# gautam-sabnis/A-Divide-and-Conquer-Strategy-for-High-Dimensional-Bayesian-Factor-Models

Measured on AMD Instinct MI355X. Metric: Gibbs iters/sec (node) at p=20k,n=1k,g=64; cov-assembly MFMA util %, higher is better.
Workload: dtype f64; 1 GPU; c3: p=19968 (P=312 x g=64), n=1000, K=30 (k=1920), rho=0.5, thin=5, burnin=0 (assembly in timed region), asm_batch=96; global_batch=1000, parallelism=shards64/gpus1

## Files before the change

### a-divide-and-conquer-strategy-for-high-dimensional-bayesian-factor-models_amd/_abi.py

```python
from __future__ import annotations

import ctypes as C
import os
from pathlib import Path

PKG_DIR = Path(__file__).resolve().parent
LIB_PATH = Path(os.environ.get("DCFM_LIB", PKG_DIR / "libdcfm.so"))

DCFM_OK = 0
DCFM_ERR_INVALID = 1
DCFM_ERR_UNSUPPORTED = 2
DCFM_ERR_HIP = 3
DCFM_ERR_RCCL = 4
DCFM_ERR_NUMERIC = 5
DCFM_ERR_ALLOC = 6
DCFM_FLAG_INJECT_DRAWS = 0x1
DCFM_FLAG_UNFUSED = 0x2
DCFM_FLAG_ONE_STREAM = 0x4
DCFM_FLAG_FLAT_PRIORITY = 0x8
DCFM_FLAG_COMM_SELF = 0x20
DCFM_FLAG_EXACT_RESIDUAL = 0x10
DCFM_FLAG_GUARD_ALL = 0x40
DCFM_FLAG_SIGMA_M2 = 0x80
DCFM_FLAG_PRECISION_MEAN = 0x100
DCFM_FLAG_PARTIAL_CORR = 0x200
DCFM_SIGMA_MEAN = 0
DCFM_SIGMA_M2 = 1
DCFM_SIGMA_SD = 2
SIGMA_MOMENTS = {"mean": DCFM_SIGMA_MEAN, "m2": DCFM_SIGMA_M2, "sd": DCFM_SIGMA_SD}

KERNEL_IDS = {
    "k_prep": 0, "k_wpass": 1, "k_zdraw": 2, "k_xred": 3, "k_xdraw": 4, "k_cpass": 5,
    "k_lambda": 6, "k_colsum": 7, "k_delta": 8, "k_save": 9, "k_assemble": 10, "rccl": 11,
    "k_xchol": 12, "k_draws": 13, "k_resid": 14,
}
K_COUNT = 15

EXPORTS = (
    "dcfm_create", "dcfm_destroy", "dcfm_last_error", "dcfm_abi_version",
    "dcfm_comm_unique_id", "dcfm_comm_init", "dcfm_comm_init_loopback", "dcfm_set_data", "dcfm_set_state",
    "dcfm_set_draws", "dcfm_run", "dcfm_synchronize", "dcfm_get_state", "dcfm_get_state_raw", "dcfm_get_sigma",
    "dcfm_get_sigma_cols", "dcfm_sigma_block", "dcfm_get_sigma_moment_cols", "dcfm_get_sigma_moment",
    "dcfm_saved_samples", "dcfm_sigma_error", "dcfm_set_profiling", "dcfm_set_profiling_mask", "dcfm_set_profiling_stride", "dcfm_get_kernel_stats",
    "dcfm_kernel_name",
    "dcfm_rng_fill", "dcfm_rng_fill_rows", "dcfm_set_data_raw", "dcfm_get_data", "dcfm_count_nonzero_columns",
    "dcfm_set_trace", "dcfm_get_trace", "dcfm_init_state", "dcfm_sigma_apply", "dcfm_sigma_eigs",
    "dcfm_sigma_solve", "dcfm_set_probes", "dcfm_get_probe_draws", "dcfm_set_precision_probes",
    "dcfm_get_precision_draws", "dcfm_get_precision_mean_cols", "dcfm_get_precision_mean",
    "dcfm_get_partial_corr_cols", "dcfm_get_partial_corr",
    "dcfm_set_loglik", "dcfm_get_loglik", "dcfm_set_predict", "dcfm_get_predict",
    "dcfm_set_missing", "dcfm_get_imputed",
)


class DcfmConfig(C.Structure):
    _fields_ = [
        ("n", C.c_int32), ("P", C.c_int32), ("g", C.c_int32), ("K", C.c_int32),
        ("rho", C.c_double),
        ("burnin", C.c_int64), ("mcmc", C.c_int64), ("thin", C.c_int64),
        ("as_", C.c_double), ("bs", C.c_double), ("df", C.c_double), ("ad1", C.c_double),
        ("bd1", C.c_double), ("ad2", C.c_double), ("bd2", C.c_double),
        ("seed", C.c_uint64),
        ("nranks", C.c_int32), ("rank", C.c_int32), ("device", C.c_int32),
        ("flags", C.c_uint32), ("asm_batch", C.c_int32), ("reserved", C.c_int32 * 7),
    ]


_DP = C.POINTER(C.c_double)


class DcfmStateView(C.Structure):
    _fields_ = [(f, _DP) for f in ("Lambda", "ps", "omega", "psi", "Plam", "X", "Z", "eta", "delta", "tauh")]


class DcfmDrawsView(C.Structure):
    _fields_ = [(f, _DP) for f in ("NZ", "NX", "NL", "Gpsi", "Gdelta", "Gps")]


class DcfmError(RuntimeError):
    def __init__(self, code: int, msg: str):
        super().__init__(f"dcfm error {code}: {msg}")
        self.code = code


_lib = None


def load_library(path: Path | None = None):
    global _lib
    if _lib is not None:
        return _lib
    p = Path(path) if path else LIB_PATH
    if not p.exists():
        raise ImportError(
            f"libdcfm.so not found at {p}: build it first (python -c 'import __graft_entry__ as g; g.build()' "
            "or make -C <pkg>/csrc). There is no CPU fallback.")
    lib = C.CDLL(str(p))
    vp = C.c_void_p
    sig = {
        "dcfm_create": (C.c_int, [C.POINTER(DcfmConfig), C.POINTER(vp)]),
        "dcfm_destroy": (None, [vp]),
        "dcfm_last_error": (C.c_char_p, [vp]),
        "dcfm_abi_version": (C.c_int, []),
        "dcfm_comm_unique_id": (C.c_int, [C.POINTER(C.c_uint8)]),
        "dcfm_comm_init": (C.c_int, [vp, C.POINTER(C.c_uint8)]),
        "dcfm_comm_init_loopback": (C.c_int, [C.POINTER(vp), C.c_int32]),
        "dcfm_set_data": (C.c_int, [vp, _DP]),
        "dcfm_set_state": (C.c_int, [vp, C.POINTER(DcfmStateView)]),
        "dcfm_set_draws": (C.c_int, [vp, C.POINTER(DcfmDrawsView), C.c_int64, C.c_int64]),
        "dcfm_run": (C.c_int, [vp, C.c_int64, C.c_int64]),
        "dcfm_synchronize": (C.c_int, [vp]),
        "dcfm_get_state": (C.c_int, [vp, C.POINTER(DcfmStateView)]),
        "dcfm_get_state_raw": (C.c_int, [vp, C.POINTER(DcfmStateView)]),
        "dcfm_get_sigma": (C.c_int, [vp, _DP]),
        "dcfm_get_sigma_cols": (C.c_int, [vp, C.c_int64, C.c_int64, _DP]),
        "dcfm_sigma_block": (C.c_int, [vp, C.POINTER(C.c_int64)]),
        "dcfm_get_sigma_moment_cols": (C.c_int, [vp, C.c_int32, C.c_int64, C.c_int64, _DP]),
        "dcfm_get_sigma_moment": (C.c_int, [vp, C.c_int32, _DP]),
        "dcfm_get_precision_mean_cols": (C.c_int, [vp, C.c_int64, C.c_int64, _DP]),
        "dcfm_get_precision_mean": (C.c_int, [vp, _DP]),
        "dcfm_get_partial_corr_cols": (C.c_int, [vp, C.c_int32, C.c_int64, C.c_int64, _DP]),
        "dcfm_get_partial_corr": (C.c_int, [vp, C.c_int32, _DP]),
        "dcfm_saved_samples": (C.c_int64, [vp]),
        "dcfm_sigma_error": (C.c_int, [vp, _DP, C.c_int32, _DP, C.c_int32, C.c_uint64, _DP]),
        "dcfm_sigma_apply": (C.c_int, [vp, _DP, C.c_int32, _DP, _DP]),
        "dcfm_sigma_eigs": (C.c_int, [vp, C.c_int32, C.c_double, C.c_int32, C.c_uint64, _DP, _DP, _DP,
                                      C.POINTER(C.c_int32)]),
        "dcfm_sigma_solve": (C.c_int, [vp, _DP, C.c_int32, C.c_double, C.c_int32, _DP, _DP, C.POINTER(C.c_int32),
                                       _DP, _DP]),
        "dcfm_set_probes": (C.c_int, [vp, _DP, C.c_int32, C.c_int64]),
        "dcfm_get_probe_draws": (C.c_int, [vp, _DP, C.POINTER(C.c_int64)]),
        "dcfm_set_precision_probes": (C.c_int, [vp, _DP, C.c_int32, C.c_int64]),
        "dcfm_get_precision_draws": (C.c_int, [vp, _DP, _DP, C.POINTER(C.c_int64)]),
        "dcfm_set_loglik": (C.c_int, [vp, C.c_int64]),
        "dcfm_get_loglik": (C.c_int, [vp, _DP, _DP, C.POINTER(C.c_int64)]),
        "dcfm_set_predict": (C.c_int, [vp, _DP, C.POINTER(C.c_uint8), C.c_int32, C.c_int64]),
        "dcfm_get_predict": (C.c_int, [vp, _DP, _DP, _DP, _DP, _DP, C.POINTER(C.c_int64)]),
        "dcfm_set_missing": (C.c_int, [vp, C.POINTER(C.c_uint8), C.c_int64]),
        "dcfm_get_imputed": (C.c_int, [vp, _DP, _DP, _DP, C.POINTER(C.c_int64)]),
        "dcfm_set_profiling": (C.c_int, [vp, C.c_int]),
        "dcfm_set_profiling_mask": (C.c_int, [vp, C.c_uint32]),
        "dcfm_set_profiling_stride": (C.c_int, [vp, C.c_int32]),
        "dcfm_get_kernel_stats": (C.c_int, [vp, _DP, C.POINTER(C.c_int64)]),
        "dcfm_kernel_name": (C.c_char_p, [C.c_int]),
        "dcfm_rng_fill": (C.c_int, [C.c_int, C.c_uint64, C.c_int, C.c_double, C.c_int32, C.c_int32,
                                    C.c_int64, C.c_int64, _DP]),
        "dcfm_rng_fill_rows": (C.c_int, [C.c_int, C.c_uint64, C.c_int, C.c_double, C.c_int32, C.c_int32,
                                         C.c_int64, C.c_int64, C.c_int32, C.c_int64, _DP]),
        "dcfm_set_data_raw": (C.c_int, [vp, _DP, C.c_int64, C.POINTER(C.c_int64), _DP, _DP]),
        "dcfm_get_data": (C.c_int, [vp, _DP]),
        "dcfm_set_trace": (C.c_int, [vp, C.c_int64]),
        "dcfm_init_state": (C.c_int, [vp]),
        "dcfm_get_trace": (C.c_int, [vp, _DP, C.POINTER(C.c_int64)]),
        "dcfm_count_nonzero_columns": (C.c_int, [C.c_int, _DP, C.c_int32, C.c_int64, C.POINTER(C.c_int32),
                                                 _DP]),
    }
    for name, (res, args) in sig.items():
        fn = getattr(lib, name)
        fn.restype = res
        fn.argtypes = args
    _lib = lib
    return lib


def check(lib, handle, code: int):
    if code != DCFM_OK:
        msg = lib.dcfm_last_error(handle)
        raise DcfmError(code, msg.decode() if msg else "")
```

### a-divide-and-conquer-strategy-for-high-dimensional-bayesian-factor-models_amd/csrc/dcfm.hip

```cpp
#include "handle.h"
#include "resid.h"

static int dalloc(dcfm_handle *h, double **p, size_t n) {
    void *q = nullptr;
    if (n == 0) n = 1;
    hipError_t e = hipMalloc(&q, n * sizeof(double));
    if (e != hipSuccess)
        return fail(h, DCFM_ERR_ALLOC, "hipMalloc(%zu doubles) failed: %s", n, hipGetErrorString(e));
    e = hipMemset(q, 0, n * sizeof(double));
    if (e != hipSuccess) return fail(h, DCFM_ERR_HIP, "hipMemset failed: %s", hipGetErrorString(e));
    h->allocs.push_back(q);
    *p = static_cast<double *>(q);
    return DCFM_OK;
}

static int round_up(int a, int b) { return (a + b - 1) / b * b; }

static double *trace_row(dcfm_handle *h, int64_t t) {
    return h->trace + trace_scratch_doubles(h->d.G) + (size_t)t * h->d.G * 4;
}

static void collect_prof(dcfm_handle *h) {
    if (h->recs.empty()) return;
    sync_all(h);
    for (auto &r : h->recs) {
        float ms = 0.f;
        if (hipEventElapsedTime(&ms, r.a, r.b) == hipSuccess) {
            h->kms[r.kid] += ms;
            h->kcnt[r.kid] += 1;
        }
        h->evpool.push_back(r.a);
        h->evpool.push_back(r.b);
    }
    h->recs.clear();
}

static std::vector<int> sigma_split(int nt, int nranks) {
    std::vector<int> Tb(nranks + 1, nt);
    Tb[0] = 0;
    const double total = (double)tri(nt);
    for (int k = 1; k < nranks; ++k) {
        const double target = total * k / nranks;
        int t = Tb[k - 1];
        while (t < nt && (double)tri(t) < target) ++t;
        if (t > Tb[k - 1] && target - (double)tri(t - 1) < (double)tri(t) - target) --t;
        Tb[k] = t;
    }
    return Tb;
}

extern "C" {

int dcfm_abi_version(void) { return DCFM_ABI_VERSION; }

const char *dcfm_last_error(const dcfm_handle *h) { return h ? h->err.c_str() : g_err.c_str(); }

const char *dcfm_kernel_name(int id) {
    static const char *names[DCFM_K_COUNT] = {"k_prep",  "k_wpass", "k_zdraw",  "k_xred",
                                              "k_xdraw", "k_cpass", "k_lambda", "k_colsum",
                                              "k_delta", "k_save",  "k_assemble", "rccl", "k_xchol",
                                              "k_draws", "k_resid"};
    return (id >= 0 && id < DCFM_K_COUNT) ? names[id] : "?";
}

static int validate_config(const dcfm_config &c) {
    if (c.n < 1 || c.P < 1 || c.g < 1 || c.K < 1)
        return fail(nullptr, DCFM_ERR_INVALID, "n, P, g, K must be >= 1");
    if (c.K > KP_MAX)
        return fail(nullptr, DCFM_ERR_UNSUPPORTED, "K = %d > %d not supported by this build", c.K, KP_MAX);
    if (!(c.rho >= 0.0 && c.rho <= 1.0)) return fail(nullptr, DCFM_ERR_INVALID, "rho must be in [0,1]");
    if (c.thin < 1 || c.mcmc < 0 || c.burnin < 0)
        return fail(nullptr, DCFM_ERR_INVALID, "thin >= 1, mcmc >= 0, burnin >= 0 required");
    if (!(c.bs > 0 && c.bd1 > 0 && c.bd2 > 0 && c.df > 0))
        return fail(nullptr, DCFM_ERR_INVALID, "bs, bd1, bd2, df must be > 0 (dc:62-65)");
    if (!(c.as_ > 0.0 && c.ad1 > 0.0 && c.ad2 > 0.0))
        return fail(nullptr, DCFM_ERR_INVALID, "as, ad1, ad2 must be > 0 (dc:62-65; got %g, %g, %g)", c.as_, c.ad1,
                    c.ad2);
    const int nranks = c.nranks < 1 ? 1 : c.nranks;
    if (c.rank < 0 || c.rank >= nranks) return fail(nullptr, DCFM_ERR_INVALID, "bad rank");
    {
        const bool fused = c.K <= KP && !(c.flags & DCFM_FLAG_UNFUSED);
        const int Gl = c.g / nranks, nxs = xsum_blocks(Gl);
        if (fused && (c.g > 1023 || nxs > 255 || Gl / nxs > 255))
            return fail(nullptr, DCFM_ERR_UNSUPPORTED, "g = %d shards (%d per rank): the fused K <= 32 chain takes at "
                        "most 1023, and a per-rank count whose odd part is below 256 (DCFM_FLAG_UNFUSED lifts "
                        "this)", c.g, Gl);
        if (!fused && c.g >= (1 << 16))
            return fail(nullptr, DCFM_ERR_UNSUPPORTED, "g = %d shards: at most %d", c.g, (1 << 16) - 1);
    }
    if (c.g % nranks)
        return fail(nullptr, DCFM_ERR_UNSUPPORTED, "g = %d not divisible by nranks = %d", c.g, nranks);
    return DCFM_OK;
}

static Dims plan(const dcfm_config &c, bool *fused, int *B, int *LDB) {
    Dims d{};
    const int nranks = c.nranks < 1 ? 1 : c.nranks;
    d.n = c.n; d.P = c.P; d.g = c.g; d.K = c.K;
    d.nranks = nranks; d.rank = c.rank;
    d.coll = (nranks > 1 || (c.flags & DCFM_FLAG_COMM_SELF)) ? 1 : 0;
    d.G = c.g / nranks;
    d.shard0 = c.rank * d.G;
    d.NP = round_up(c.n, 128);
    d.PP = round_up(c.P, 32);
    d.p = c.P * c.g;
    d.kp = padded_width(c.K);
    d.rho = c.rho; d.sr = std::sqrt(c.rho); d.s1r = std::sqrt(1.0 - c.rho);
    d.as_ = c.as_; d.bs = c.bs; d.df = c.df; d.ad1 = c.ad1; d.bd1 = c.bd1; d.ad2 = c.ad2; d.bd2 = c.bd2;
    d.seed = c.seed;
    d.inject = (c.flags & DCFM_FLAG_INJECT_DRAWS) ? 1 : 0;
    *fused = d.kp == KP && !(c.flags & DCFM_FLAG_UNFUSED);
    const bool packed = d.coll && *fused;
    d.sgap = packed ? KP * KP + d.NP * KP : 0;
    d.xstride = packed ? d.G * KP + KP * KP + d.NP * KP : d.kp * d.kp;
    *B = c.asm_batch > 0 ? c.asm_batch : 32;
    *LDB = round_up(*B * d.K, ASM_KC);
    return d;
}

static int create_streams_and_events(dcfm_handle *h) {
    const dcfm_config &c = h->cfg;
    HIPC(h, hipSetDevice(c.device));
    int prio_lo = 0, prio_hi = 0;
    if (!(c.flags & DCFM_FLAG_FLAT_PRIORITY)) HIPC(h, hipDeviceGetStreamPriorityRange(&prio_lo, &prio_hi));
    HIPC(h, hipStreamCreateWithPriority(&h->stream, hipStreamNonBlocking, prio_hi));
    {
        if (c.flags & DCFM_FLAG_ONE_STREAM) {
            h->side = h->sasm = h->sdraw = h->stream;
        } else {
            HIPC(h, hipStreamCreateWithPriority(&h->side, hipStreamNonBlocking, prio_hi));
            HIPC(h, hipStreamCreateWithPriority(&h->sdraw, hipStreamNonBlocking, prio_lo));
            HIPC(h, hipStreamCreateWithPriority(&h->sasm, hipStreamNonBlocking, prio_lo));
        }
    }
    for (hipEvent_t *e : {&h->e_lam, &h->e_prep, &h->e_xchol, &h->e_batch, &h->e_free[0], &h->e_free[1], &h->e_drawn[0],
                          &h->e_used[0], &h->e_drawn[1], &h->e_used[1]})
        HIPC(h, hipEventCreateWithFlags(e, hipEventDisableTiming));
    return DCFM_OK;
}

static int alloc_buffers(dcfm_handle *h) {
    const dcfm_config &c = h->cfg;
    const int nranks = c.nranks;
    void *q = nullptr;
    HIPC(h, hipMalloc(&q, sizeof(int)));
    h->allocs.push_back(q);
    h->nan_dev = static_cast<int *>(q);
    HIPC(h, hipMemset(h->nan_dev, 0, sizeof(int)));
    HIPC(h, hipHostMalloc(&q, sizeof(int), hipHostMallocDefault));
    h->nan_host = static_cast<int *>(q);
    *h->nan_host = 0;
    const Dims &d = h->d;
    Bufs &b = h->b;
    const size_t G = d.G, NP = d.NP, PP = d.PP, g = d.g, p = d.p, KP = d.kp;
    TRY(dalloc(h, &b.Y, G * NP * PP));
    TRY(dalloc(h, &b.yy, G * PP));
    TRY(dalloc(h, &b.Lam, G * PP * KP));
    TRY(dalloc(h, &b.omega, G * PP));
    TRY(dalloc(h, &b.ps, G * PP));
    TRY(dalloc(h, &b.psi, G * PP * KP));
    TRY(dalloc(h, &b.Plam, G * PP * KP));
    TRY(dalloc(h, &b.X, NP * KP));
    TRY(dalloc(h, &b.Z, G * NP * KP));
    TRY(dalloc(h, &b.delta, 2 * g * KP));
    TRY(dalloc(h, &b.tau, 2 * g * KP));
    TRY(dalloc(h, &b.W, G * NP * KP));
    TRY(dalloc(h, &b.A, G * KP * KP));
    TRY(dalloc(h, &b.ZM, G * 4 * KP * KP));
    TRY(dalloc(h, &b.Sp, G * NP * KP));
    if (d.sgap) {
        const size_t msg = (size_t)d.xstride;
        TRY(dalloc(h, &b.sloc, msg));
        b.xa = b.sloc + (size_t)G * KP;
        b.xin = b.xa + KP * KP;
        TRY(dalloc(h, &b.msg_all, (size_t)nranks * msg));
        b.sall = b.msg_all;
        b.xa_all = b.msg_all + (size_t)G * KP;
        b.xall = b.xa_all + KP * KP;
    } else {
        TRY(dalloc(h, &b.xin, NP * KP));
        if (d.coll) { TRY(dalloc(h, &b.xall, (size_t)nranks * NP * KP)); } else b.xall = b.xin;
        TRY(dalloc(h, &b.xa, KP * KP));
        TRY(dalloc(h, &b.xa_all, (size_t)nranks * KP * KP));
    }
    TRY(dalloc(h, &b.XM, 2 * KP * KP));
    TRY(dalloc(h, &b.agree, 3));
    {
        double *rf = nullptr;
        TRY(dalloc(h, &rf, (G * (PP / 32) + 1) / 2));
        b.rflag = reinterpret_cast<int *>(rf);
    }
    TRY(dalloc(h, &b.xpart, (size_t)G * KP * KP));
    {
        double *tk = nullptr;
        TRY(dalloc(h, &tk, 1));
        b.ticket = reinterpret_cast<unsigned *>(tk);
        double *sy = nullptr;
        TRY(dalloc(h, &sy, SYNC_ZM + G));
        b.sync = reinterpret_cast<unsigned long long *>(sy);
    }
    TRY(dalloc(h, &b.C, G * PP * KP));
    TRY(dalloc(h, &b.E, G * KP * KP));
    TRY(dalloc(h, &b.cpart, G * PP * KP));
    if (!d.sgap) {
        TRY(dalloc(h, &b.sloc, G * KP));
        if (d.coll) { TRY(dalloc(h, &b.sall, g * KP)); } else b.sall = b.sloc;
    }
    TRY(dalloc(h, &b.Lb[0], p * (size_t)b.LDB));
    TRY(dalloc(h, &b.Lb[1], p * (size_t)b.LDB));
    TRY(dalloc(h, &b.wsum[0], p));
    TRY(dalloc(h, &b.wsum[1], p));
    {
        const int nt = (d.p + ASM_TILE - 1) / ASM_TILE;
        h->Tb = sigma_split(nt, nranks);
        b.T0 = h->Tb[c.rank];
        b.T1 = h->Tb[c.rank + 1];
    }
    TRY(dalloc(h, &b.Sigma, (size_t)(tri(b.T1) - tri(b.T0)) * ASM_TILE * ASM_TILE));
    if (c.flags & DCFM_FLAG_SIGMA_M2) {
        TRY(dalloc(h, &b.Sigma2, (size_t)(tri(b.T1) - tri(b.T0)) * ASM_TILE * ASM_TILE));
    }
    if (c.flags & DCFM_FLAG_PRECISION_MEAN)
        TRY(dalloc(h, &h->pm.Prec, (size_t)(tri(b.T1) - tri(b.T0)) * ASM_TILE * ASM_TILE));
    if (c.flags & DCFM_FLAG_PARTIAL_CORR) {
        TRY(dalloc(h, &h->pc.PC, (size_t)(tri(b.T1) - tri(b.T0)) * ASM_TILE * ASM_TILE));
        TRY(dalloc(h, &h->pc.PC2, (size_t)(tri(b.T1) - tri(b.T0)) * ASM_TILE * ASM_TILE));
    }
    if (c.flags & (DCFM_FLAG_PRECISION_MEAN | DCFM_FLAG_PARTIAL_CORR)) {
        PrecMean &pm = h->pm;
        pm.KH = round_up(h->B * d.K, ASM_KC);
        TRY(dalloc(h, &pm.pfac, p * 4 * (size_t)pm.KH));
        TRY(dalloc(h, &pm.pscr, precision_mean_scratch_doubles(d.g, d.K, h->B)));
        HIPC(h, precision_mean_setup());
    }
    if (c.flags & (DCFM_FLAG_SIGMA_M2 | DCFM_FLAG_PRECISION_MEAN | DCFM_FLAG_PARTIAL_CORR)) {
        TRY(dalloc(h, &b.wslot[0], p * (size_t)h->B));
        TRY(dalloc(h, &b.wslot[1], p * (size_t)h->B));
    }
    if (h->fused && !d.inject) TRY(dalloc(h, &b.ldraw, (size_t)lam_gen_doubles(d)));
    if (!d.inject && !h->fused) {
        const size_t K = c.K, n = c.n, P = c.P;
        const size_t nz = K * n * g, nx = K * n, nl = K * P * g, gpsi = P * K * g, gdel = K * g, gps = P * g;
        const size_t per_it = nz + nx + nl + gpsi + gdel + gps;
        h->DB = (int)std::max<size_t>(1, std::min<size_t>(8, (size_t(2) << 30) / (2 * per_it * sizeof(double))));
        const size_t sz[6] = {nz, nx, nl, gpsi, gdel, gps};
        for (int i = 0; i < 6; ++i) h->draw_iter_sz[i] = sz[i];
        double *gm = nullptr;
        TRY(dalloc(h, &gm, 2 * (size_t)h->DB * per_it));
        for (int sl = 0; sl < 2; ++sl) {
            DrawsDev &G = h->gen[sl];
            G.NZ = gm; gm += nz * h->DB;
            G.NX = gm; gm += nx * h->DB;
            G.NL = gm; gm += nl * h->DB;
            G.Gpsi = gm; gm += gpsi * h->DB;
            G.Gdelta = gm; gm += gdel * h->DB;
            G.Gps = gm; gm += gps * h->DB;
            G.first_iter = -1;
            G.n_iter = h->DB;
        }
    }
    return DCFM_OK;
}

static int upload_tile_list(dcfm_handle *h) {
    Bufs &b = h->b;
    constexpr int SB = 8;
    std::vector<int2> tl;
    for (int rb0 = b.T0; rb0 < b.T1; rb0 += SB) {
        const int rb1 = std::min(b.T1, rb0 + SB);
        for (int cb0 = 0; cb0 < rb1; cb0 += SB)
            for (int ti = rb0; ti < rb1; ++ti)
                for (int tj = cb0; tj < std::min(cb0 + SB, ti + 1); ++tj) tl.push_back(make_int2(ti, tj));
    }
    if ((int64_t)tl.size() != tri(b.T1) - tri(b.T0))
        return fail(h, DCFM_ERR_INVALID, "assembly tile list: %zu tiles for %lld", tl.size(),
                    (long long)(tri(b.T1) - tri(b.T0)));
    b.ntiles = (int)tl.size();
    void *q = nullptr;
    HIPC(h, hipMalloc(&q, std::max<size_t>(1, tl.size()) * sizeof(int2)));
    h->allocs.push_back(q);
    b.tiles = static_cast<int2 *>(q);
    if (!tl.empty()) HIPC(h, hipMemcpy(b.tiles, tl.data(), tl.size() * sizeof(int2), hipMemcpyHostToDevice));
    return DCFM_OK;
}

static int fill_delta_tau_ones(dcfm_handle *h) {
    std::vector<double> ones(2 * (size_t)h->d.g * h->d.kp, 1.0);
    HIPC(h, hipMemcpy(h->b.delta, ones.data(), ones.size() * sizeof(double), hipMemcpyHostToDevice));
    HIPC(h, hipMemcpy(h->b.tau, ones.data(), ones.size() * sizeof(double), hipMemcpyHostToDevice));
    return DCFM_OK;
}

int dcfm_create(const dcfm_config *cfg, dcfm_handle **out) {
    if (!cfg || !out) return fail(nullptr, DCFM_ERR_INVALID, "null argument");
    *out = nullptr;
    const dcfm_config &c = *cfg;
    TRY(validate_config(c));
    int ndev = 0;
    hipError_t e = hipGetDeviceCount(&ndev);
    if (e != hipSuccess || ndev < 1)
        return fail(nullptr, DCFM_ERR_HIP, "no HIP device available (%s)", hipGetErrorString(e));
    if (c.device < 0 || c.device >= ndev) return fail(nullptr, DCFM_ERR_INVALID, "bad device %d", c.device);

    dcfm_handle *h = new dcfm_handle();
    h->d = plan(c, &h->fused, &h->B, &h->b.LDB);
    h->cfg = c;
    h->cfg.nranks = h->d.nranks;
    int rc = create_streams_and_events(h);
    if (rc == DCFM_OK) rc = alloc_buffers(h);
    if (rc == DCFM_OK) rc = upload_tile_list(h);
    if (rc == DCFM_OK) rc = fill_delta_tau_ones(h);
    if (rc != DCFM_OK) {
        g_err = h->err;
        dcfm_destroy(h);
        return rc;
    }
    *out = h;
    return DCFM_OK;
}

void dcfm_destroy(dcfm_handle *h) {
    if (!h) return;
    (void)hipSetDevice(h->cfg.device);
    if (h->stream) sync_all(h);
    for (auto &r : h->recs) { (void)hipEventDestroy(r.a); (void)hipEventDestroy(r.b); }
    for (auto e : h->evpool) (void)hipEventDestroy(e);
    for (hipEvent_t e : {h->e_lam, h->e_prep, h->e_xchol, h->e_batch, h->e_free[0], h->e_free[1], h->e_drawn[0],
                         h->e_drawn[1], h->e_used[0], h->e_used[1]})
        if (e) (void)hipEventDestroy(e);
    if (h->lp_ready) (void)hipEventDestroy(h->lp_ready);
    if (h->lp_done) (void)hipEventDestroy(h->lp_done);
    if (h->comm_asm) ncclCommDestroy(h->comm_asm);
    if (h->comm_side) ncclCommDestroy(h->comm_side);
    if (h->comm) ncclCommDestroy(h->comm);
    for (void *q : h->allocs) (void)hipFree(q);
    if (h->nan_host) (void)hipHostFree(h->nan_host);
    if (h->draws_mem) (void)hipFree(h->draws_mem);
    if (h->trace) (void)hipFree(h->trace);
    if (h->probe_mem) (void)hipFree(h->probe_mem);
    if (h->prec_mem) (void)hipFree(h->prec_mem);
    if (h->ll_mem) (void)hipFree(h->ll_mem);
    if (h->pred_mem) (void)hipFree(h->pred_mem);
    if (h->imp_mem) (void)hipFree(h->imp_mem);
    if (h->sasm && h->sasm != h->stream) (void)hipStreamDestroy(h->sasm);
    if (h->side && h->side != h->stream) (void)hipStreamDestroy(h->side);
    if (h->sdraw && h->sdraw != h->stream) (void)hipStreamDestroy(h->sdraw);
    if (h->stream) (void)hipStreamDestroy(h->stream);
    delete h;
}

static int flush_batch(dcfm_handle *h) {
    if (h->batch == 0) return DCFM_OK;
    Dims &d = h->d;
    Bufs &b = h->b;
    const int lb = h->lb;
    HIPC(h, hipEventRecord(h->e_batch, h->stream));
    HIPC(h, hipStreamWaitEvent(h->sasm, h->e_batch, 0));
    if (d.coll) {
        KTimer t(h, DCFM_K_COMM, h->sasm);
        const size_t rows = (size_t)d.G * d.P;
        if (!h->loop) NCCLC(h, ncclGroupStart());
        int rc = coll_allgather(h, CH_ASM, b.Lb[lb] + (size_t)d.rank * rows * b.LDB, b.Lb[lb], rows * b.LDB,
                                h->sasm);
        if (rc == DCFM_OK)
            rc = coll_allgather(h, CH_ASM, b.wsum[lb] + (size_t)d.rank * rows, b.wsum[lb], rows, h->sasm);
        if (rc == DCFM_OK && b.wslot[lb])
            rc = coll_allgather(h, CH_ASM, b.wslot[lb] + (size_t)d.rank * rows * h->B, b.wslot[lb], rows * h->B,
                                h->sasm);
        if (!h->loop) NCCLC(h, ncclGroupEnd());
        if (rc) return rc;
    }
    const int used = h->batch * d.K, kext = round_up(used, 4), kstage = round_up(used, ASM_KC);
    const double effsamp = (double)h->cfg.mcmc / (double)h->cfg.thin;
    if (kstage > used)
        HIPC(h, hipMemset2DAsync(b.Lb[lb] + used, (size_t)b.LDB * sizeof(double), 0, (size_t)(kstage - used) * sizeof(double),
                                 (size_t)d.p, h->sasm));
    {
        KTimer t(h, DCFM_K_ASSEMBLE, h->sasm);
        launch_assemble(d, b, b.Lb[lb], b.wsum[lb], kext, 1.0 / effsamp, h->sasm);
        if (b.Sigma2) launch_assemble_m2(d, b, b.Lb[lb], b.wslot[lb], h->batch, h->B, 1.0 / effsamp, h->sasm);
        if (h->pm.pfac) launch_precision_panels(d, b, h->pm, b.Lb[lb], b.wslot[lb], h->batch, h->B, h->sasm);
        if (h->pm.Prec) launch_precision_mean(d, b, h->pm, b.wslot[lb], h->batch, h->B, 1.0 / effsamp, h->sasm);
        if (h->pc.PC) launch_partial_corr(d, b, h->pm, h->pc, b.wslot[lb], h->batch, h->B, 1.0 / effsamp, h->sasm);
    }
    HIPC(h, hipGetLastError());
    HIPC(h, hipMemsetAsync(b.wsum[lb], 0, (size_t)d.p * sizeof(double), h->sasm));
    HIPC(h, hipEventRecord(h->e_free[lb], h->sasm));
    h->asm_pending[lb] = true;
    h->lb ^= 1;
    h->batch = 0;
    return DCFM_OK;
}

static int check_run_args(dcfm_handle *h, int64_t first_iter, int64_t n_iter) {
    if (!h) return fail(h, DCFM_ERR_INVALID, "null handle");
    if (!h->have_data || !h->have_state) return fail(h, DCFM_ERR_INVALID, "set_data and set_state first");
    if (first_iter < 1 || n_iter < 0) return fail(h, DCFM_ERR_INVALID, "iterations are 1-based");
    if (h->d.coll && !h->comm_ok) return fail(h, DCFM_ERR_INVALID, "dcfm_comm_init first (nranks > 1 or COMM_SELF)");
    if (h->d.inject) {
        if (!h->dr.NZ) return fail(h, DCFM_ERR_INVALID, "INJECT_DRAWS set but no draws");
        if (first_iter < h->dr.first_iter || first_iter + n_iter > h->dr.first_iter + h->dr.n_iter)
            return fail(h, DCFM_ERR_INVALID, "iterations [%lld,%lld) not covered by injected draws",
                        (long long)first_iter, (long long)(first_iter + n_iter));
    }
    return DCFM_OK;
}

struct DeltaTau { const double *delta_in, *tau_in; double *delta_out, *tau_out; };
static DeltaTau delta_tau(const dcfm_handle *h) {
    const size_t nkg = (size_t)h->d.g * h->d.kp, in = h->cur * nkg, out = (1 - h->cur) * nkg;
    return {h->b.delta + in, h->b.tau + in, h->b.delta + out, h->b.tau + out};
}

static void iteration_done(dcfm_handle *h) {
    h->cur ^= 1;
    if (h->trace_n < h->trace_cap) {
        launch_trace(h->d, h->b, delta_tau(h).tau_in, h->trace, trace_row(h, h->trace_n), h->stream);
        h->trace_n += 1;
    }
}

static bool saved_iteration(const dcfm_handle *h, int64_t it) { return it % h->cfg.thin == 0 && it > h->cfg.burnin; }

#ifndef DCFM_LAM_SAVE
#define DCFM_LAM_SAVE 1
#endif
static bool lambda_saves(const dcfm_handle *h) {
    return DCFM_LAM_SAVE && h->d.kp == KP && !(h->cfg.flags & DCFM_FLAG_EXACT_RESIDUAL);
}

static int open_batch(dcfm_handle *h) {
    if (h->batch == 0 && h->asm_pending[h->lb]) {
        HIPC(h, hipStreamWaitEvent(h->stream, h->e_free[h->lb], 0));
        h->asm_pending[h->lb] = false;
    }
    return DCFM_OK;
}

static int loading_rows(dcfm_handle *h, const DrawsDev &dr, int64_t it, bool lamgen) {
    const Dims &d = h->d;
    const Bufs &b = h->b;
    hipStream_t s = h->stream;
    const bool exact = h->cfg.flags & DCFM_FLAG_EXACT_RESIDUAL;
    const double kappa_max = exact ? HUGE_VAL : (h->cfg.flags & DCFM_FLAG_GUARD_ALL) ? 0.0 : KAPPA_IDENTITY_MAX;
    SaveArgs sv;
    if (lambda_saves(h) && saved_iteration(h, it)) {
        TRY(open_batch(h));
        sv.Lb = b.Lb[h->lb]; sv.wsum = b.wsum[h->lb]; sv.wslot = b.wslot[h->lb];
        sv.LDB = b.LDB; sv.slot = h->batch; sv.B = h->B;
    }
    {
        KTimer t(h, DCFM_K_LAMBDA, s);
        launch_lambda(d, b, dr, it, delta_tau(h).tau_in, h->plam_valid ? b.Plam : nullptr, s, lamgen, kappa_max, sv);
    }
    if (exact) {
        KTimer t(h, DCFM_K_RESID, s);
        launch_resid(d, b, dr, it, s, lamgen);
    } else if (d.kp != KP) {
        KTimer t(h, DCFM_K_RESID, s);
        launch_resid_flagged(d, b, dr, it, s);
    }
    h->plam_valid = false;
    if (h->imp.nmiss) {
        KTimer t(h, DCFM_K_SAVE, s);
        const bool acc = saved_iteration(h, it) && h->imp_n < h->imp_cap;
        launch_impute(d, b, h->imp, it, acc, s);
        if (acc) h->imp_n += 1;
    }
    return DCFM_OK;
}

static int save_sample(dcfm_handle *h, int64_t it) {
    if (!saved_iteration(h, it)) return DCFM_OK;
    const Bufs &b = h->b;
    hipStream_t s = h->stream;
    const bool ksave = !lambda_saves(h);
    if (ksave) TRY(open_batch(h));
    if (ksave || h->probe_n < h->probe_cap || h->prec_n < h->prec_cap || h->ll_n < h->ll_cap ||
        h->pred_n < h->pred_cap) {
        KTimer t(h, DCFM_K_SAVE, s);
        if (ksave) launch_save(h->d, b, b.Lb[h->lb], b.wsum[h->lb], h->batch, s, b.wslot[h->lb], h->B);
        if (h->probe_n < h->probe_cap) launch_probes(h->d, b, h->probes, h->probe_n++, s);
        if (h->prec_n < h->prec_cap) launch_precision(h->d, b, h->prec, h->prec_n++, s);
        if (h->ll_n < h->ll_cap) launch_loglik(h->d, b, h->ll, h->ll_n++, s);
        if (h->pred_n < h->pred_cap) launch_predict(h->d, b, h->pred, h->pred_n++, s);
    }
    HIPC(h, hipGetLastError());
    h->batch += 1;
    h->saved += 1;
    if (h->batch == h->B) TRY(flush_batch(h));
    return DCFM_OK;
}

struct FusedSchedule {
    dcfm_handle *h;
    const Dims &d;
    const Bufs &b;
    hipStream_t s;
    bool delta_pending = false;
    const DrawsDev &draws() const { return d.inject ? h->dr : h->gen[0]; }

    int step(int64_t it) {
        const DrawsDev &dr = draws();
        const bool lamgen = !d.inject;
        { KTimer t(h, DCFM_K_WPASS, s); launch_wcol(d, b, dr, it, true, delta_pending, true, ++h->wc_ops, s, lamgen); }
        if (d.coll) {
            { KTimer t(h, DCFM_K_XRED, s); launch_xred(d, b, s); }
            KTimer t(h, DCFM_K_COMM, s);
            TRY(coll_allgather(h, CH_MAIN, b.sloc, b.msg_all, (size_t)d.xstride, s));
        }
        {
            KTimer t(h, DCFM_K_XDRAW, s);
            if (d.coll) launch_xdraw_mr(d, b, dr, it, ++h->xm_ops, s);
            else launch_xdraw(d, b, dr, it, s, true);
        }
        {
            KTimer t(h, DCFM_K_CPASS, s);
            const DeltaTau dt = delta_tau(h);
            if (delta_pending) launch_cpass(d, b, s, dr, dt.delta_in, dt.tau_in, dt.delta_out, dt.tau_out, it - 1);
            else launch_cpass(d, b, s);
        }
        HIPC(h, hipGetLastError());
        if (delta_pending) iteration_done(h);
        TRY(loading_rows(h, dr, it, lamgen));
        delta_pending = true;
        return DCFM_OK;
    }

    int tail(int64_t last_iter) {
        if (!delta_pending) return DCFM_OK;
        KTimer t(h, DCFM_K_DELTA, s);
        launch_wcol(d, b, h->dr, last_iter, false, true, false, 0, s);
        if (d.coll) TRY(coll_allgather(h, CH_MAIN, b.sloc, b.msg_all, (size_t)d.xstride, s));
        const DeltaTau dt = delta_tau(h);
        launch_delta(d, b, draws(), last_iter, dt.delta_in, dt.tau_in, dt.delta_out, dt.tau_out, s);
        HIPC(h, hipGetLastError());
        iteration_done(h);
        return DCFM_OK;
    }
};

struct DrawBatches {
    dcfm_handle *h;
    int64_t end_iter;
    int64_t batch0, batch_n = 0;
    int slot = -1;
    int generate(int64_t b0, int busy) {
        hipStream_t sd = h->sdraw;
        const int64_t nb = std::min<int64_t>(h->DB, end_iter - b0);
        for (int sl = 0; sl < 2; ++sl)
            if (h->gen_first[sl] == b0 && h->gen_n[sl] >= nb) return sl;
        int sl = busy >= 0 ? 1 - busy : (h->gen_first[0] <= h->gen_first[1] ? 0 : 1);
        hipError_t e = hipSuccess;
        if (h->used_pending[sl]) {
            e = hipStreamWaitEvent(sd, h->e_used[sl], 0);
            h->used_pending[sl] = false;
        }
        for (int64_t it = b0; e == hipSuccess && it < b0 + nb; ++it) {
            const size_t o = (size_t)(it - b0);
            DrawsDev v = h->gen[sl];
            const size_t *sz = h->draw_iter_sz;
            v.NZ += o * sz[0]; v.NX += o * sz[1]; v.NL += o * sz[2];
            v.Gpsi += o * sz[3]; v.Gdelta += o * sz[4]; v.Gps += o * sz[5];
            v.first_iter = it; v.n_iter = 1;
            KTimer t(h, DCFM_K_DRAWS, sd);
            launch_draws(h->d, v, it, sd);
        }
        if (e == hipSuccess) e = hipEventRecord(h->e_drawn[sl], sd);
        if (e != hipSuccess) {
            fail(h, DCFM_ERR_HIP, "draws batch at iteration %lld: %s", (long long)b0, hipGetErrorString(e));
            return -1;
        }
        h->gen[sl].first_iter = b0;
        h->gen_first[sl] = b0;
        h->gen_n[sl] = nb;
        return sl;
    }

    int acquire(int64_t it) {
        if (it != batch0 + batch_n) return DCFM_OK;
        batch0 = it;
        batch_n = std::min<int64_t>(h->DB, end_iter - it);
        slot = generate(it, -1);
        if (slot < 0) return DCFM_ERR_HIP;
        HIPC(h, hipStreamWaitEvent(h->stream, h->e_drawn[slot], 0));
        if (it + batch_n < end_iter && generate(it + batch_n, slot) < 0) return DCFM_ERR_HIP;
        return DCFM_OK;
    }

    int release(int64_t it) {
        if (it != batch0 + batch_n - 1) return DCFM_OK;
        HIPC(h, hipEventRecord(h->e_used[slot], h->stream));
        h->used_pending[slot] = true;
        return DCFM_OK;
    }
};

struct SideSchedule {
    dcfm_handle *h;
    const Dims &d;
    const Bufs &b;
    DrawBatches gen;

    int step(int64_t it) {
        hipStream_t s = h->stream, ss = h->side;
        const size_t KW = d.kp;
        if (!d.inject) TRY(gen.acquire(it));
        const DrawsDev &dr = d.inject ? h->dr : h->gen[gen.slot];
        HIPC(h, hipStreamWaitEvent(ss, h->e_lam, 0));
        { KTimer t(h, DCFM_K_PREP, ss); launch_prep(d, b, ss); }
        HIPC(h, hipEventRecord(h->e_prep, ss));
        { KTimer t(h, DCFM_K_XCHOL, ss); launch_asum(d, b, ss); }
        if (d.coll) {
            KTimer t(h, DCFM_K_COMM, ss);
            TRY(coll_allgather(h, CH_SIDE, b.xa, b.xa_all, KW * KW, ss));
        }
        { KTimer t(h, DCFM_K_XCHOL, ss); launch_xchol(d, b, ss); }
        HIPC(h, hipEventRecord(h->e_xchol, ss));
        { KTimer t(h, DCFM_K_WPASS, s);  launch_wpass(d, b, s); }
        HIPC(h, hipStreamWaitEvent(s, h->e_prep, 0));
        { KTimer t(h, DCFM_K_ZDRAW, s);  launch_zdraw(d, b, dr, it, s); }
        { KTimer t(h, DCFM_K_XRED, s);   launch_xred(d, b, s); }
        if (d.coll) {
            KTimer t(h, DCFM_K_COMM, s);
            TRY(coll_allgather(h, CH_MAIN, b.xin, b.xall, (size_t)d.NP * KW, s));
        }
        HIPC(h, hipStreamWaitEvent(s, h->e_xchol, 0));
        { KTimer t(h, DCFM_K_XDRAW, s); launch_xdraw(d, b, dr, it, s, false); }
        { KTimer t(h, DCFM_K_CPASS, s); launch_cpass(d, b, s); }
        TRY(loading_rows(h, dr, it, false));
        HIPC(h, hipEventRecord(h->e_lam, s));
        { KTimer t(h, DCFM_K_COLSUM, s); launch_colsum(d, b, s); }
        if (d.coll) {
            KTimer t(h, DCFM_K_COMM, s);
            TRY(coll_allgather(h, CH_MAIN, b.sloc, b.sall, (size_t)d.G * KW, s));
        }
        {
            KTimer t(h, DCFM_K_DELTA, s);
            const DeltaTau dt = delta_tau(h);
            launch_delta(d, b, dr, it, dt.delta_in, dt.tau_in, dt.delta_out, dt.tau_out, s);
        }
        if (!d.inject) TRY(gen.release(it));
        iteration_done(h);
        return DCFM_OK;
    }
};

int dcfm_run(dcfm_handle *h, int64_t first_iter, int64_t n_iter) {
    TRY(check_run_args(h, first_iter, n_iter));
    HIPC(h, hipSetDevice(h->cfg.device));
    hipStream_t s = h->stream;
    const int64_t end_iter = first_iter + n_iter;
    FusedSchedule fused{h, h->d, h->b, s};
    SideSchedule side{h, h->d, h->b, DrawBatches{h, end_iter, first_iter}};
    if (!h->fused) HIPC(h, hipEventRecord(h->e_lam, s));
    for (int64_t it = first_iter; it < end_iter; ++it) {
        TRY(h->fused ? fused.step(it) : side.step(it));
        HIPC(h, hipGetLastError());
        TRY(save_sample(h, it));
    }
    if (h->fused) TRY(fused.tail(end_iter - 1));
    TRY(flush_batch(h));
    launch_finite(h->d, h->b, delta_tau(h).tau_in, h->nan_dev, s);
    HIPC(h, hipGetLastError());
    HIPC(h, hipMemcpyAsync(h->nan_host, h->nan_dev, sizeof(int), hipMemcpyDeviceToHost, s));
    if (h->prof) collect_prof(h);
    return DCFM_OK;
}

int dcfm_set_trace(dcfm_handle *h, int64_t capacity) {
    if (!h || capacity < 0) return fail(h, DCFM_ERR_INVALID, "set_trace: bad argument");
    HIPC(h, hipSetDevice(h->cfg.device));
    HIPC(h, hipStreamSynchronize(h->stream));
    if (h->trace) (void)hipFree(h->trace);
    h->trace = nullptr;
    h->trace_cap = h->trace_n = 0;
    if (capacity == 0) return DCFM_OK;
    const size_t nd = trace_scratch_doubles(h->d.G) + (size_t)capacity * h->d.G * 4;
    if (hipMalloc(&h->trace, nd * sizeof(double)) != hipSuccess)
        return fail(h, DCFM_ERR_ALLOC, "set_trace: %lld rows", (long long)capacity);
    HIPC(h, hipMemset(h->trace, 0, trace_scratch_doubles(h->d.G) * sizeof(double)));
    h->trace_cap = capacity;
    return DCFM_OK;
}

int dcfm_get_trace(dcfm_handle *h, double *out, int64_t *count) {
    if (!h || !count) return fail(h, DCFM_ERR_INVALID, "get_trace: null argument");
    HIPC(h, hipSetDevice(h->cfg.device));
    HIPC(h, hipStreamSynchronize(h->stream));
    *count = h->trace_n;
    if (out && h->trace_n) {
        const int G = h->d.G;
        std::vector<double> rows((size_t)h->trace_n * G * 4);
        HIPC(h, hipMemcpy(rows.data(), trace_row(h, 0), rows.size() * sizeof(double), hipMemcpyDeviceToHost));
        for (int64_t t = 0; t < h->trace_n; ++t)
            for (int q = 0; q < 4; ++q) {
                double acc = 0.0;
                for (int m = 0; m < G; ++m) acc += rows[((size_t)t * G + m) * 4 + q];
                out[t * 4 + q] = acc;
            }
    }
    return DCFM_OK;
}

int dcfm_synchronize(dcfm_handle *h) {
    if (!h) return fail(h, DCFM_ERR_INVALID, "null handle");
    HIPC(h, hipSetDevice(h->cfg.device));
    HIPC(h, hipStreamSynchronize(h->stream));
    HIPC(h, hipStreamSynchronize(h->side));
    HIPC(h, hipStreamSynchronize(h->sdraw));
    HIPC(h, hipStreamSynchronize(h->sasm));
    return numeric_status(h);
}

int64_t dcfm_saved_samples(const dcfm_handle *h) { return h ? h->saved : -1; }

int dcfm_set_profiling(dcfm_handle *h, int enable) {
    return dcfm_set_profiling_mask(h, enable ? 0xFFFFFFFFu : 0u);
}

int dcfm_set_profiling_mask(dcfm_handle *h, uint32_t mask) {
    if (!h) return fail(h, DCFM_ERR_INVALID, "null handle");
    collect_prof(h);
    h->prof_mask = mask;
    h->prof_stride = 1;
    std::fill(h->prof_seq, h->prof_seq + DCFM_K_COUNT, (int64_t)0);
    const bool enable = mask != 0;
    h->prof = enable;
    if (enable) {
        std::fill(h->kms, h->kms + DCFM_K_COUNT, 0.0);
        std::fill(h->kcnt, h->kcnt + DCFM_K_COUNT, 0);
    }
    return DCFM_OK;
}

int dcfm_set_profiling_stride(dcfm_handle *h, int32_t stride) {
    if (!h) return fail(h, DCFM_ERR_INVALID, "null handle");
    if (stride < 1) return fail(h, DCFM_ERR_INVALID, "profiling stride %d < 1", (int)stride);
    h->prof_stride = stride;
    std::fill(h->prof_seq, h->prof_seq + DCFM_K_COUNT, (int64_t)0);
    return DCFM_OK;
}

int dcfm_get_kernel_stats(dcfm_handle *h, double ms[DCFM_K_COUNT], int64_t launches[DCFM_K_COUNT]) {
    if (!h) return fail(h, DCFM_ERR_INVALID, "null handle");
    collect_prof(h);
    for (int k = 0; k < DCFM_K_COUNT; ++k) {
        if (ms) ms[k] = h->kms[k];
        if (launches) launches[k] = h->kcnt[k];
    }
    return DCFM_OK;
}

int dcfm_rng_fill(int device, uint64_t seed, int kind, double shape, int32_t site, int32_t shard,
                  int64_t iter, int64_t count, double *out) {
    if (count < 0) return fail(nullptr, DCFM_ERR_INVALID, "rng_fill: bad argument");
    return dcfm_rng_fill_rows(device, seed, kind, shape, site, shard, iter, (count + 31) / 32, 32, count, out);
}

int dcfm_rng_fill_rows(int device, uint64_t seed, int kind, double shape, int32_t site, int32_t shard,
                       int64_t iter, int64_t rows, int32_t width, int64_t count, double *out) {
    if (!out || count < 0 || rows < 0 || width < 1 || width > (1 << 23) || count > rows * (int64_t)width ||
        (kind != 0 && kind != 1) || (kind == 1 && !(shape > 0.0)))
        return fail(nullptr, DCFM_ERR_INVALID, "rng_fill: bad argument");
    hipError_t e = hipSetDevice(device);
    if (e != hipSuccess) return fail(nullptr, DCFM_ERR_HIP, "hipSetDevice: %s", hipGetErrorString(e));
    void *q = nullptr;
    e = hipMalloc(&q, std::max<int64_t>(count, 1) * sizeof(double));
    if (e != hipSuccess) return fail(nullptr, DCFM_ERR_ALLOC, "hipMalloc: %s", hipGetErrorString(e));
    launch_rng_fill(seed, kind, shape, site, shard, iter, count, width, static_cast<double *>(q), nullptr);
    e = hipGetLastError();
    if (e == hipSuccess) e = hipMemcpy(out, q, count * sizeof(double), hipMemcpyDeviceToHost);
    (void)hipFree(q);
    if (e != hipSuccess) return fail(nullptr, DCFM_ERR_HIP, "rng_fill: %s", hipGetErrorString(e));
    return DCFM_OK;
}

}
```

### a-divide-and-conquer-strategy-for-high-dimensional-bayesian-factor-models_amd/csrc/dcfm_internal.h

```cpp
#pragma once
#include <hip/hip_runtime.h>
#include <stdint.h>

namespace dcfm {

constexpr int KP = 32;
constexpr int KP_MAX = 128;
constexpr int padded_width(int K) { return K <= 32 ? 32 : (K <= 64 ? 64 : 128); }
constexpr int ASM_TILE = 128;
__host__ __device__ constexpr int etile(int nbw, int Kc, int I) { return Kc * nbw - Kc * (Kc - 1) / 2 + (I - Kc); }
__host__ __device__ constexpr int etile_index(int nbw, int R, int Cc) {
    return (2 * etile(nbw, R >> 4, Cc >> 4) + ((R & 15) >> 3)) * 128 + 2 * ((Cc & 15) + 16 * (R & 3)) +
           (((R & 15) >> 2) & 1);
}
constexpr int ASM_KC = 16;
inline int cdiv(int a, int b) { return (a + b - 1) / b; }

struct Dims {
    int n, P, g, K, G;
    int NP, PP;
    int shard0;
    int nranks, rank;
    int coll;
    int p;
    int kp;
    double rho, sr, s1r;
    double as_, bs, df, ad1, bd1, ad2, bd2;
    uint64_t seed;
    int inject;
    int sgap, xstride;
};

struct DrawsDev {
    const double *NZ, *NX, *NL, *Gpsi, *Gdelta, *Gps;
    int64_t first_iter, n_iter;
};

struct LamDraws { const double *NL, *Gpsi, *Gps; };
struct SaveArgs {
    double *Lb = nullptr, *wsum = nullptr, *wslot = nullptr;
    int LDB = 0, slot = 0, B = 0;
};
#ifndef DCFM_LAM_GEN_BLOCKS
#define DCFM_LAM_GEN_BLOCKS 160
#endif
constexpr int LAM_GEN_THREADS = 256, LAM_GEN_BLOCKS = DCFM_LAM_GEN_BLOCKS;
struct LamGen { double *NL, *Gpsi, *Gps; int n_ps, n_psi, n_all, b_total; };
inline int lam_gen_doubles(const Dims &d) { return 2 * d.G * d.P * d.K + d.G * d.P; }
inline LamGen lam_gen_plan(const Dims &d, double *base) {
    const int T = LAM_GEN_THREADS, GP = d.G * d.P;
    LamGen g;
    g.NL = base;
    g.Gpsi = base + (size_t)GP * d.K;
    g.Gps = base + 2 * (size_t)GP * d.K;
    g.n_ps = GP;
    g.n_psi = GP + GP * d.K;
    g.n_all = g.n_psi + GP * ((d.K + 1) / 2);
    const int full = (g.n_all + T - 1) / T;
    g.b_total = full < LAM_GEN_BLOCKS ? full : LAM_GEN_BLOCKS;
    return g;
}

struct Bufs {
    double *Y, *yy, *Lam, *omega, *ps, *psi, *Plam, *X, *Z, *delta, *tau;
    double *ldraw;
    double *W, *A, *ZM, *Sp, *xin, *xall, *C, *E, *cpart, *sloc, *sall;
    double *Lb[2], *wsum[2], *Sigma;
    double *wslot[2], *Sigma2;
    double *xa, *xa_all, *XM;
    double *xpart;
    unsigned *ticket;
    unsigned long long *sync;
    double *msg_all;
    double *agree;
    int *rflag;
    int2 *tiles;
    int ntiles, LDB;
    int T0, T1;
};

inline LamDraws lam_draws_at(const Dims &d, const Bufs &b, const DrawsDev &dr, int64_t iter, bool gen) {
    if (gen) {
        const LamGen g = lam_gen_plan(d, b.ldraw);
        return {g.NL, g.Gpsi, g.Gps};
    }
    const size_t row0 = ((size_t)(iter - dr.first_iter) * d.g + d.shard0) * d.P;
    return {dr.NL + row0 * d.K, dr.Gpsi + row0 * d.K, dr.Gps + row0};
}

constexpr int XSUM_BLOCKS = 8;
constexpr int TRACE_SLICES = 16;
constexpr int PROBE_NV_MAX = 32, PROBE_SLICES_MAX = 32, PROBE_FAN = 8;
inline int probe_slices(int G) { return G >= 256 ? 1 : (256 / G < PROBE_SLICES_MAX ? 256 / G : PROBE_SLICES_MAX); }
struct Probes {
    const double *V;
    double *part, *term, *gterm, *draws;
    unsigned *ticket;
    int nv, slices;
    size_t slot;
};
__host__ __device__ constexpr int precision_tiles(int K, int nv) { return ((K + nv + 15) / 16) * ((K + nv + 15) / 16 + 1) / 2; }
inline int precision_slices(int G, int P, int K, int nv) {
    const int wp = (K + nv + 15) / 16 * 16, rows = wp / 2 > 8 ? wp / 2 : 8, cap = P / rows > 1 ? P / rows : 1;
    return probe_slices(G) < cap ? probe_slices(G) : cap;
}
struct Precision {
    const double *V;
    double *part, *gram, *term, *gterm, *rsum, *xs, *draws;
    unsigned *ticket;
    int nv, slices;
    size_t slot, lds;
};
struct LogLik {
    Precision pr;
    double *T, *sq, *binv, *hsum, *sinv, *draws;
    size_t slot, lds;
};
struct Predict {
    Precision pr;
    unsigned char *obs;
    double *sinv, *qd, *work, *coef, *sum, *sum2, *cvsum, *draws;
    int T, Tp, wc;
};
struct Impute {
    int nmiss, ncol;
    const int *row, *col, *perm, *colptr, *cols;
    double *vcsc, *yyobs, *smu, *smu2, *snv;
};
struct PrecMean {
    double *Prec, *pfac, *pscr;
    int KH;
};
struct PartialCorr {
    double *PC, *PC2;
};
constexpr int SYNC_ZM = 2 + 256;
__host__ __device__ inline int xsum_blocks(int G) {
    if (G <= XSUM_BLOCKS) return 1;
    int chunk = 1;
    while (G / chunk > XSUM_BLOCKS && (G / chunk) % 2 == 0) chunk *= 2;
    return G / chunk;
}

__host__ __device__ inline long long tri(long long t) { return t * (t + 1) / 2; }
__host__ __device__ inline int sig_tile_off(int u, int v, int g, int w, int lane) {
    return ((((w * 4 + u) * 4 + v) * 2 + (g >> 1)) * 64 + lane) * 2 + (g & 1);
}
__host__ __device__ inline size_t sig_off(int a, int b, int T0) {
    const int ta = a / ASM_TILE, tb = b / ASM_TILE, ra = a % ASM_TILE, cb = b % ASM_TILE, rr = ra & 15;
    return (size_t)(tri(ta) - tri(T0) + tb) * ASM_TILE * ASM_TILE +
           sig_tile_off((ra >> 4) & 3, (cb >> 4) & 3, rr >> 2, 2 * (ra >> 6) + (cb >> 6), (rr & 3) * 16 + (cb & 15));
}
__host__ __device__ inline long long win_lo(long long c, long long R0, long long R1) {
    return (c >= R0 && c < R1) ? 0 : (c < R0 ? R0 : R1);
}
__host__ __device__ inline long long win_off(long long c, long long c0, long long R0, long long R1) {
    const long long na = (c < R0 ? c : R0) - c0;
    const long long b0 = c0 > R0 ? c0 : R0, b1 = c < R1 ? c : R1;
    return (na > 0 ? na : 0) * (R1 - R0) + (b1 > b0 ? b1 - b0 : 0) * R1;
}

void launch_prep(const Dims &d, const Bufs &b, hipStream_t s);
void launch_wpass(const Dims &d, const Bufs &b, hipStream_t s);
void launch_zdraw(const Dims &d, const Bufs &b, const DrawsDev &dr, int64_t iter, hipStream_t s);
void launch_xred(const Dims &d, const Bufs &b, hipStream_t s);
void launch_wcol(const Dims &d, const Bufs &b, const DrawsDev &dr, int64_t iter, bool ops, bool colsum, bool wpass,
                 unsigned long long ops_epoch, hipStream_t s, bool lamgen = false);
void launch_xdraw_mr(const Dims &d, const Bufs &b, const DrawsDev &dr, int64_t iter, unsigned long long xm_epoch,
                     hipStream_t s);
void launch_asum(const Dims &d, const Bufs &b, hipStream_t s);
void launch_xchol(const Dims &d, const Bufs &b, hipStream_t s);
void launch_xdraw(const Dims &d, const Bufs &b, const DrawsDev &dr, int64_t iter, hipStream_t s,
                  bool from_shards = false);
void launch_cpass(const Dims &d, const Bufs &b, hipStream_t s, const DrawsDev &dr = DrawsDev{},
                  const double *delta_in = nullptr, const double *tau_in = nullptr, double *delta_out = nullptr,
                  double *tau_out = nullptr, int64_t delta_iter = 0);
void launch_lambda(const Dims &d, const Bufs &b, const DrawsDev &dr, int64_t iter,
                   const double *tau_cur, const double *plam_src, hipStream_t s, bool gen, double kappa_max,
                   const SaveArgs &sv = SaveArgs{});
void launch_colsum(const Dims &d, const Bufs &b, hipStream_t s);
void launch_resid(const Dims &d, const Bufs &b, const DrawsDev &dr, int64_t iter, hipStream_t s, bool gen);
void launch_resid_flagged(const Dims &d, const Bufs &b, const DrawsDev &dr, int64_t iter, hipStream_t s);
void launch_delta(const Dims &d, const Bufs &b, const DrawsDev &dr, int64_t iter,
                  const double *delta_in, const double *tau_in, double *delta_out,
                  double *tau_out, hipStream_t s);
void launch_save(const Dims &d, const Bufs &b, double *Lb, double *wsum, int slot, hipStream_t s,
                 double *wslot = nullptr, int B = 0);
void launch_assemble(const Dims &d, const Bufs &b, const double *Lb, const double *wsum, int kext,
                     double inv_eff, hipStream_t s);
void launch_assemble_m2(const Dims &d, const Bufs &b, const double *Lb, const double *wslot, int nslots, int B,
                        double inv_eff, hipStream_t s);
size_t precision_mean_scratch_doubles(int g, int K, int B);
hipError_t precision_mean_setup();
void launch_precision_panels(const Dims &d, const Bufs &b, const PrecMean &pm, const double *Lb, const double *wslot,
                             int nslots, int B, hipStream_t s);
void launch_precision_mean(const Dims &d, const Bufs &b, const PrecMean &pm, const double *wslot, int nslots, int B,
                           double inv_eff, hipStream_t s);
void launch_pc_mean(const Dims &d, const Bufs &b, const PrecMean &pm, int nslots, double inv_eff, double *PC,
                    hipStream_t s);
void launch_partial_corr(const Dims &d, const Bufs &b, const PrecMean &pm, const PartialCorr &pc, const double *wslot,
                         int nslots, int B, double inv_eff, hipStream_t s);
void launch_sigma_pack(const double *S, const double *S2, int which, double rs, int p, int T0, int T1, int c0,
                       int nc, double *out, hipStream_t s, const double *diag = nullptr);
void launch_sigma_unpack(const double *recv, int p, int c0, int nc, const int *Tb, const long long *base,
                         int nranks, double *out, hipStream_t s);
void launch_eta(const Dims &d, const Bufs &b, double *eta_out, hipStream_t s);
int sigma_err_splits(int p);
void launch_sigma_err(const double *S, int p, const double *U, int R, const double *sdiag, const double *v,
                      int T0, int T1, bool first, double *y, double *fro, double *tru, double *out,
                      hipStream_t s);
size_t sigma_apply_scratch(int T0, int T1, int nv);
void launch_sigma_apply(const double *S, int p, int T0, int T1, const double *V, int nv, double *scratch, double *Y,
                        hipStream_t s);
void launch_nnz_cols(const double *Y, int n, long long p, int *nnz, hipStream_t s);
void launch_stdize(const Dims &d, const double *Yraw, const long long *cols, double *Y, double *yy, double *sd,
                   int *bad, double *mean_inv, hipStream_t s);
inline size_t trace_scratch_doubles(int G) { return (size_t)G * TRACE_SLICES * 4 + (G + 1) / 2; }
void launch_trace(const Dims &d, const Bufs &b, const double *tau_cur, double *scratch, double *row, hipStream_t s);
void launch_probes(const Dims &d, const Bufs &b, const Probes &pr, int64_t s, hipStream_t st);
void launch_precision(const Dims &d, const Bufs &b, const Precision &pr, int64_t s, hipStream_t st);
void launch_precision_terms(const Dims &d, const Bufs &b, const Precision &pr, double *binv, double *out, hipStream_t st);
size_t precision_ticket_doubles(const Dims &d);
size_t precision_scratch_doubles(const Dims &d, int nv);
void precision_scratch_carve(const Dims &d, int nv, double *mem, Precision &pr);
hipError_t precision_setup();
void launch_precision_masked(const Dims &d, const Bufs &b, const Precision &pr, const unsigned char *obs, double *sinv,
                             double *draw, hipStream_t st);
void launch_predict(const Dims &d, const Bufs &b, const Predict &pd, int64_t s, hipStream_t st);
void launch_impute(const Dims &d, const Bufs &b, const Impute &im, int64_t iter, bool acc, hipStream_t s);
void launch_loglik(const Dims &d, const Bufs &b, const LogLik &ll, int64_t s, hipStream_t st);
void launch_init_state(const Dims &d, const Bufs &b, hipStream_t s);
void launch_draws(const Dims &d, const DrawsDev &dr, int64_t iter, hipStream_t s);
void launch_finite(const Dims &d, const Bufs &b, const double *tau_cur, int *flag, hipStream_t s);
void launch_sum_slices(const double *src, int ns, size_t count, double *dst, hipStream_t s);
void launch_rng_fill(uint64_t seed, int kind, double shape, int site, int shard, int64_t iter,
                     int64_t count, int width, double *out, hipStream_t s);

namespace wide {
void launch_prep(const Dims &d, const Bufs &b, hipStream_t s);
void launch_xchol(const Dims &d, const Bufs &b, hipStream_t s);
void launch_zdraw(const Dims &d, const Bufs &b, const DrawsDev &dr, int64_t iter, hipStream_t s);
void launch_xdraw(const Dims &d, const Bufs &b, const DrawsDev &dr, int64_t iter, hipStream_t s);
void launch_lambda(const Dims &d, const Bufs &b, const DrawsDev &dr, int64_t iter, const double *tau_cur,
                   const double *plam_src, hipStream_t s, double kappa_max);
void launch_delta(const Dims &d, const Bufs &b, const DrawsDev &dr, int64_t iter, const double *delta_in,
                  const double *tau_in, double *delta_out, double *tau_out, hipStream_t s);
}

}
```

### a-divide-and-conquer-strategy-for-high-dimensional-bayesian-factor-models_amd/csrc/handle.h

```cpp
#pragma once
#include "../../include/dcfm.h"
#include "dcfm_internal.h"

#include <rccl/rccl.h>

#include <algorithm>
#include <chrono>
#include <cmath>
#include <condition_variable>
#include <memory>
#include <mutex>
#include <cstdarg>
#include <cstdio>
#include <cstdlib>
#include <cstring>
#include <string>
#include <vector>

using namespace dcfm;

#pragma GCC visibility push(hidden)

struct ProfRec { int kid; hipEvent_t a, b; };
struct LoopGroup;

struct dcfm_handle {
    dcfm_config cfg{};
    Dims d{};
    Bufs b{};
    DrawsDev dr{};
    hipStream_t stream = nullptr;
    hipStream_t side = nullptr;
    hipStream_t sdraw = nullptr;
    hipStream_t sasm = nullptr;
    ncclComm_t comm = nullptr, comm_side = nullptr, comm_asm = nullptr;
    bool comm_ok = false;
    std::shared_ptr<LoopGroup> loop;
    std::vector<int> Tb;
    hipEvent_t lp_ready = nullptr, lp_done = nullptr;
    hipEvent_t e_lam = nullptr, e_prep = nullptr, e_xchol = nullptr, e_batch = nullptr,
               e_free[2] = {nullptr, nullptr}, e_drawn[2] = {nullptr, nullptr}, e_used[2] = {nullptr, nullptr};
    bool fused = false;
    bool plam_valid = false;
    unsigned long long wc_ops = 0;
    unsigned long long xm_ops = 0;
    bool asm_pending[2] = {false, false};
    int cur = 0;
    int lb = 0;
    int B = 16;
    int batch = 0;
    int64_t saved = 0;
    bool have_data = false, have_state = false;
    int *nan_dev = nullptr;
    int *nan_host = nullptr;
    std::string err;
    std::vector<void *> allocs;
    double *draws_mem = nullptr;
    DrawsDev gen[2] = {};
    int64_t gen_first[2] = {-1, -1}, gen_n[2] = {0, 0};
    bool used_pending[2] = {false, false};
    int DB = 1;
    size_t draw_iter_sz[6] = {};
    double *trace = nullptr;
    int64_t trace_cap = 0, trace_n = 0;
    double *probe_mem = nullptr;
    Probes probes{};
    int64_t probe_cap = 0, probe_n = 0;
    double *prec_mem = nullptr;
    Precision prec{};
    int64_t prec_cap = 0, prec_n = 0;
    double *ll_mem = nullptr;
    LogLik ll{};
    int64_t ll_cap = 0, ll_n = 0;
    double *pred_mem = nullptr;
    Predict pred{};
    int64_t pred_cap = 0, pred_n = 0;
    void *imp_mem = nullptr;
    Impute imp{};
    int64_t imp_cap = 0, imp_n = 0;
    PrecMean pm{};
    PartialCorr pc{};
    bool prof = false;
    uint32_t prof_mask = 0;
    int prof_stride = 1;
    int64_t prof_seq[DCFM_K_COUNT] = {};
    std::vector<ProfRec> recs;
    std::vector<hipEvent_t> evpool;
    double kms[DCFM_K_COUNT] = {};
    int64_t kcnt[DCFM_K_COUNT] = {};
};

inline std::string g_err;

inline int fail(dcfm_handle *h, int code, const char *fmt, ...) {
    char buf[1024];
    va_list ap;
    va_start(ap, fmt);
    vsnprintf(buf, sizeof buf, fmt, ap);
    va_end(ap);
    if (h) h->err = buf; else g_err = buf;
    return code;
}

#define HIPC(h, x)                                                                        \
    do {                                                                                  \
        hipError_t e_ = (x);                                                              \
        if (e_ != hipSuccess)                                                             \
            return fail(h, DCFM_ERR_HIP, "%s failed: %s (%s:%d)", #x, hipGetErrorString(e_), \
                        __FILE__, __LINE__);                                              \
    } while (0)

#define TRY(x) do { if (int rc_ = (x)) return rc_; } while (0)

#define NCCLC(h, x)                                                                      \
    do {                                                                                  \
        ncclResult_t r_ = (x);                                                            \
        if (r_ != ncclSuccess)                                                            \
            return fail(h, DCFM_ERR_RCCL, "%s failed: %s", #x, ncclGetErrorString(r_));   \
    } while (0)

enum { CH_MAIN = 0, CH_SIDE = 1, CH_ASM = 2 };

int coll_allgather(dcfm_handle *h, int ch, const double *send, double *recv, size_t count, hipStream_t s);
int coll_gather(dcfm_handle *h, const double *send, double *recv, const std::vector<long long> &base,
                const std::vector<long long> &cnt, int root, hipStream_t s);
int coll_allreduce_sum(dcfm_handle *h, int ch, double *buf, size_t count, hipStream_t s);
int agree(dcfm_handle *h, int code);

inline hipEvent_t get_event(dcfm_handle *h) {
    if (!h->evpool.empty()) {
        hipEvent_t e = h->evpool.back();
        h->evpool.pop_back();
        return e;
    }
    hipEvent_t e;
    if (hipEventCreateWithFlags(&e, hipEventDisableSystemFence) != hipSuccess) return nullptr;
    return e;
}

struct KTimer {
    dcfm_handle *h;
    int kid;
    hipStream_t s;
    hipEvent_t a = nullptr;
    KTimer(dcfm_handle *h_, int k, hipStream_t s_) : h(h_), kid(k), s(s_) {
        if (h->prof && (h->prof_mask >> k & 1u) && h->prof_seq[k]++ % h->prof_stride == 0) {
            a = get_event(h);
            if (a) (void)hipEventRecord(a, s);
        }
    }
    ~KTimer() {
        if (h->prof && a) {
            hipEvent_t b = get_event(h);
            if (b) {
                (void)hipEventRecord(b, s);
                h->recs.push_back({kid, a, b});
            }
        }
    }
};

inline void sync_all(dcfm_handle *h) {
    (void)hipStreamSynchronize(h->stream);
    if (h->side) (void)hipStreamSynchronize(h->side);
    if (h->sdraw) (void)hipStreamSynchronize(h->sdraw);
    if (h->sasm) (void)hipStreamSynchronize(h->sasm);
}

inline int numeric_status(dcfm_handle *h) {
    if (h->nan_host && *h->nan_host)
        return fail(h, DCFM_ERR_NUMERIC, "non-finite sampler state (NaN / Inf in Lambda, ps, omega, X or tau) "
                                         "after dcfm_run; set_state / init_state to restart");
    return DCFM_OK;
}

void impute_drop(dcfm_handle *h);

inline uint64_t splitmix64(uint64_t &x) {
    uint64_t z = (x += 0x9E3779B97F4A7C15ull);
    z = (z ^ (z >> 30)) * 0xBF58476D1CE4E5B9ull;
    z = (z ^ (z >> 27)) * 0x94D049BB133111EBull;
    return z ^ (z >> 31);
}

#pragma GCC visibility pop
```

### a-divide-and-conquer-strategy-for-high-dimensional-bayesian-factor-models_amd/csrc/handoff.h

```cpp
#pragma once
#include <hip/hip_runtime.h>

namespace dcfm {

__device__ __forceinline__ void st_agent(double *p, double v) {
    __hip_atomic_store(p, v, __ATOMIC_RELAXED, __HIP_MEMORY_SCOPE_AGENT);
}
__device__ __forceinline__ double ld_agent(const double *p) {
    return __hip_atomic_load(const_cast<double *>(p), __ATOMIC_RELAXED, __HIP_MEMORY_SCOPE_AGENT);
}

__device__ __forceinline__ void stores_done() {
    asm volatile("s_waitcnt vmcnt(0)" ::: "memory");
    __syncthreads();
}

__device__ __forceinline__ void signal_count(unsigned long long *ctr) {
    stores_done();
    if (threadIdx.x == 0) __hip_atomic_fetch_add(ctr, 1ull, __ATOMIC_RELAXED, __HIP_MEMORY_SCOPE_AGENT);
}
__device__ __forceinline__ void wait_count(unsigned long long *ctr, unsigned long long target) {
    if (threadIdx.x == 0)
        while (__hip_atomic_load(ctr, __ATOMIC_RELAXED, __HIP_MEMORY_SCOPE_AGENT) < target) __builtin_amdgcn_s_sleep(1);
    __syncthreads();
}

__device__ __forceinline__ bool last_arrival(unsigned *ticket, unsigned count, unsigned *flag) {
    stores_done();
    if (threadIdx.x == 0) {
        const bool last =
            __hip_atomic_fetch_add(ticket, 1u, __ATOMIC_RELAXED, __HIP_MEMORY_SCOPE_AGENT) == count - 1;
        if (last) __hip_atomic_store(ticket, 0u, __ATOMIC_RELAXED, __HIP_MEMORY_SCOPE_AGENT);
        *flag = last ? 1u : 0u;
    }
    __syncthreads();
    const bool last = *flag != 0u;
    __syncthreads();
    return last;
}

}
```

### a-divide-and-conquer-strategy-for-high-dimensional-bayesian-factor-models_amd/csrc/kernels.hip

```cpp
#include "dcfm_internal.h"
#include "philox.h"
#include "linalg.h"
#include "handoff.h"
#include "wstamp.h"
#include "zx_ops.h"
#include "ypass.h"
#include "draws.h"
#include "zdraw.h"
#include "delta.h"
#include "lambda.h"

#include <algorithm>

namespace dcfm {

__global__ __launch_bounds__(256) void k_prep(Dims d, const double *__restrict__ Lam,
                                              const double *__restrict__ omega,
                                              double *__restrict__ A, double *__restrict__ ZM) {
    __shared__ double smem[PREP_SMEM];
    prep_shard(d, Lam, omega, A, ZM, blockIdx.x, smem);
}

template <int KW>
__global__ __launch_bounds__(256) void k_wpass(Dims d, const double *__restrict__ Y,
                                               const double *__restrict__ Lam,
                                               const double *__restrict__ omega,
                                               double *__restrict__ W) {
    const int w = xcd_remap(blockIdx.x, gridDim.x);
    wpass_tile<KW>(d, Y, Lam, omega, W, w / (KW / 32), w % (KW / 32));
}

template <int ZT>
__global__ __launch_bounds__(ZT) __attribute__((amdgpu_waves_per_eu(ZT == ZTHREADS ? 4 : 2))) void k_zdraw(Dims d, const double *__restrict__ W,
                                               const double *__restrict__ ZM,
                                               const double *__restrict__ X,
                                               double *__restrict__ Z, double *__restrict__ Sp,
                                               DrawsDev dr, int64_t iter) {
    __shared__ double smem[ZDRAW_SMEM];
    zdraw_tile<ZT>(d, W, ZM, X, Z, Sp, dr, iter, xcd_remap(blockIdx.x, gridDim.x), smem);
}

__global__ __launch_bounds__(256) void k_xred(Dims d, const double *__restrict__ Sp,
                                              double *__restrict__ xin) {
    const size_t total = (size_t)d.NP * d.kp;
    const size_t e = blockIdx.x * (size_t)blockDim.x + threadIdx.x;
    if (e >= total) return;
    xin[e] = tree_sum(Sp + e, d.G, total);
}

__global__ __launch_bounds__(256) void k_asum(Dims d, const double *__restrict__ A,
                                              double *__restrict__ xa) {
    const int e = blockIdx.x * 256 + threadIdx.x;
    const int kk = d.kp * d.kp;
    if (e >= kk) return;
    xa[e] = tree_sum(A + e, d.G, (size_t)kk);
}

__global__ __launch_bounds__(256) void k_xchol(Dims d, const double *__restrict__ xa_all,
                                               double *__restrict__ XM) {
    __shared__ double smem[XCHOL_SMEM];
    for (int e = threadIdx.x; e < KP * KP; e += 256) {
        xprec_store(d, smem, e, tree_sum(xa_all + e, d.nranks, (size_t)d.xstride));
    }
    __syncthreads();
    xchol_factor(d, XM, smem);
}

__device__ __forceinline__ void xdraw_chunks(int nsrc, int &nch, int &chunk) {
    chunk = 1;
    while (nsrc / chunk > 4 && (nsrc / chunk) % 2 == 0) chunk *= 2;
    nch = nsrc / chunk;
    if (nch > 4) { nch = 1; chunk = nsrc; }
}
constexpr int XD_ROWS = 4;
#ifndef DCFM_XD_SPREAD
#define DCFM_XD_SPREAD 1
#endif
constexpr bool XD_SPREAD = DCFM_XD_SPREAD;
constexpr int XD_LDS = 2 * KP * (KP + 1) + 4 * 4 * 64 * 2 + 4 * 64 * 2;
constexpr int XD_SMEM = XD_LDS > XCHOL_SMEM ? XD_LDS : XCHOL_SMEM;
__global__ __launch_bounds__(1024) void k_xdraw(Dims d, const double *__restrict__ src, int nsrc, size_t sstride,
                                                double *__restrict__ XM,
                                                double *__restrict__ X, DrawsDev dr, int64_t iter, int xroles,
                                                const double *__restrict__ xa, unsigned long long *xm_ctr,
                                                unsigned long long xm_target) {
    __shared__ double smem[XD_SMEM];
    int blk = blockIdx.x;
    if (xroles & 1) {
        if (blk == 0) {
            for (int e = threadIdx.x; e < KP * KP; e += 1024)
                xprec_store(d, smem, e, d.nranks > 1 ? tree_sum(xa + e, d.nranks, (size_t)d.xstride) : xa[e]);
            __syncthreads();
            xchol_factor<true>(d, XM, smem);
            signal_count(xm_ctr);
            return;
        }
        blk -= 1;
    }
    double (*Ms)[KP][KP + 1] = reinterpret_cast<double (*)[KP][KP + 1]>(smem);
    d2 (*part)[4][64] = reinterpret_cast<d2 (*)[4][64]>(smem + 2 * KP * (KP + 1));
    d2 (*evs)[64] = reinterpret_cast<d2 (*)[64]>(smem + 2 * KP * (KP + 1) + 4 * 4 * 64 * 2);
    const int lane = threadIdx.x & 63, w = threadIdx.x >> 6, c = lane & 15, q = lane >> 4;
    const int tw = w & 3, sw = w >> 2;
    const int i0 = blk * XD_ROWS, i = i0 + c;
    const bool live = c < XD_ROWS && i < d.n;
    const size_t stride = sstride;
    int nch, chunk;
    xdraw_chunks(nsrc, nch, chunk);
    d2 sv[4], ev[4];
    if (w == 0 && d.inject) {
        const double *nx = dr.NX + ((size_t)(iter - dr.first_iter) * d.n + (live ? i : 0)) * d.K;
#pragma unroll
        for (int t = 0; t < 4; ++t) {
            const int kk = 8 * t + 2 * q;
            ev[t].x = (live && kk < d.K) ? nx[kk] : 0.0;
            ev[t].y = (live && kk + 1 < d.K) ? nx[kk + 1] : 0.0;
        }
    } else if (w == 0 && !XD_SPREAD) {
        const Rng rng(d.seed);
#pragma unroll
        for (int t = 0; t < 4; ++t) {
            const int kk = 8 * t + 2 * q;
            double n0 = 0.0, n1 = 0.0;
            if (live && kk < d.K) rng.normal2(SITE_X, 0u, (uint32_t)i, (uint32_t)(4 * t + q), (uint32_t)iter, n0, n1);
            ev[t].x = n0;
            ev[t].y = (kk + 1 < d.K) ? n1 : 0.0;
        }
    }
    double xmv[2] = {0.0, 0.0};
    if (!(xroles & 1)) {
#pragma unroll
        for (int u = 0; u < 2; ++u) xmv[u] = XM[threadIdx.x + 1024 * u];
    }
    auto draw = [&] {
        if (!XD_SPREAD || d.inject || w >= 4) return;
        const int kk = 8 * w + 2 * q;
        double n0 = 0.0, n1 = 0.0;
        if (live && kk < d.K) Rng(d.seed).normal2(SITE_X, 0u, (uint32_t)i, (uint32_t)(4 * w + q), (uint32_t)iter, n0, n1);
        evs[w][lane] = d2{n0, (kk + 1 < d.K) ? n1 : 0.0};
    };
    if (sw < nch) {
        if (chunk >= 2) {
            constexpr int NPART = 16 / XD_ROWS;
            const int np = (chunk & (chunk - 1)) ? 1 : (chunk < NPART ? chunk : NPART), per = chunk / np;
            const int rr = c % XD_ROWS, h = c / XD_ROWS;
            const bool rl = i0 + rr < d.n && h < np;
            const double *p = src + (size_t)(sw * chunk + (h < np ? h : 0) * per) * stride +
                              (size_t)(i0 + rr < d.n ? i0 + rr : i0) * KP + 8 * tw + 2 * q;
            d2 v = tree_sum_f<d2, 8, 10>(per, [&](int rk) {
                return rl ? *reinterpret_cast<const d2 *>(p + (size_t)rk * stride) : d2{0.0, 0.0};
            }, draw);
            for (int o = 1; o < np; o <<= 1) {
                d2 u;
                u.x = __shfl_down(v.x, o * XD_ROWS, 16);
                u.y = __shfl_down(v.y, o * XD_ROWS, 16);
                v.x = v.x + u.x;
                v.y = v.y + u.y;
            }
            part[sw][tw][lane] = h == 0 ? v : d2{0.0, 0.0};
        } else {
            const double *p = src + (size_t)sw * chunk * stride + (size_t)(live ? i : i0) * KP + 8 * tw + 2 * q;
            const d2 v = live ? *reinterpret_cast<const d2 *>(p) : d2{0.0, 0.0};
            draw();
            part[sw][tw][lane] = v;
        }
    }
    if (xroles & 1) {
        wait_count(xm_ctr, xm_target);
#pragma unroll
        for (int u = 0; u < 2; ++u) xmv[u] = ld_agent(XM + threadIdx.x + 1024 * u);
    }
#pragma unroll
    for (int u = 0; u < 2; ++u) {
        const int e = threadIdx.x + 1024 * u;
        const int mat = e / (KP * KP), rem = e % (KP * KP);
        Ms[mat][rem / KP][rem % KP] = xmv[u];
    }
    __syncthreads();
    if (w > 0) return;
    if (XD_SPREAD && !d.inject) {
#pragma unroll
        for (int t = 0; t < 4; ++t) ev[t] = evs[t][lane];
    }
#pragma unroll
    for (int t = 0; t < 4; ++t) {
        TreeSum<d2, 3> ts;
        for (int k = 0; k < nch; ++k) ts.push(part[k][t][lane]);
        sv[t] = ts.total();
    }
    d4 ax[2];
    ax[0] = ax[1] = d4{0.0, 0.0, 0.0, 0.0};
#pragma unroll
    for (int t = 0; t < 4; ++t)
#pragma unroll
        for (int e = 0; e < 2; ++e) {
            const int kk = 8 * t + 2 * q + e;
            const double se = e ? sv[t].y : sv[t].x, ee = e ? ev[t].y : ev[t].x;
#pragma unroll
            for (int mt = 0; mt < 2; ++mt) {
                ax[mt] = mfma16x16x4(Ms[0][16 * mt + c][kk], se, ax[mt]);
                ax[mt] = mfma16x16x4(Ms[1][16 * mt + c][kk], ee, ax[mt]);
            }
        }
    if (!live) return;
    double *Xr = X + (size_t)i * KP;
#pragma unroll
    for (int mt = 0; mt < 2; ++mt)
#pragma unroll
        for (int g = 0; g < 4; ++g) {
            const int k = 16 * mt + q + 4 * g;
            Xr[k] = (k < d.K) ? ax[mt][g] : 0.0;
        }
}

constexpr int CP_WAVES = 4;
template <int KW, bool PS = false>
__global__ __launch_bounds__(64 * CP_WAVES) __attribute__((amdgpu_waves_per_eu(3))) void k_cpass(Dims d, const double *__restrict__ Y,
                                                              const double *__restrict__ X,
                                                              const double *__restrict__ Z,
                                                              double *__restrict__ C, double *__restrict__ E,
                                                              DrawsDev dr, const double *__restrict__ sall,
                                                              DeltaArgs da, int ndel) {
    __shared__ double red[CP_WAVES][32][33];
    const int nbc = gridDim.x - ndel;
    if constexpr (KW == KP) {
        if ((int)blockIdx.x >= nbc) {
            const int m = (blockIdx.x - nbc) * CP_WAVES + (threadIdx.x >> 6);
            if (m < d.g)
                delta_shard<KP>(d, sall, da.delta_in, da.tau_in, da.delta_out, da.tau_out, dr, da.iter, m, threadIdx.x & 63);
            return;
        }
    }
    const int nt = (d.PP + KW) >> 5, nkt = KW / 32;
    int w = xcd_remap(blockIdx.x, nbc);
    const int par = PS ? (w & 1) : 0;
    if (PS) w >>= 1;
    const int kt = w % nkt, m = (w / nkt) / nt, tile = (w / nkt) % nt;
    const int wave = threadIdx.x >> 6, lane = threadIdx.x & 63;
    const int c0 = tile * 32;
    const bool isE = c0 >= d.PP;
    const int te = isE ? (c0 - d.PP) >> 5 : 0;
    const int r = lane & 15, q = lane >> 4;
    const double *Yp = Y + (size_t)m * d.NP * d.PP + c0 + 2 * r;
    constexpr bool ETA = KW > KP;
    const double *Xs = ETA ? X + (size_t)m * d.NP * KW : X;
    const double *Xp = Xs + 32 * kt + 2 * r;
    const double *Zp = Z + (size_t)m * d.NP * KW + 32 * kt + 2 * r;
    const double *Xa = Xs + 32 * te + 2 * r;
    const double *Za = Z + (size_t)m * d.NP * KW + 32 * te + 2 * r;
    const int nsw = d.NP / (4 * CP_WAVES);
    d4 acc[2][2];
#pragma unroll
    for (int a = 0; a < 2; ++a)
#pragma unroll
        for (int b = 0; b < 2; ++b) acc[a][b] = d4{0.0, 0.0, 0.0, 0.0};
    if (!isE) cpass_wave<KW, false, false, PS>(d, Yp, Xp, Zp, Xa, Za, wave * nsw, nsw, q, acc, par);
    else if (te == kt) cpass_wave<KW, true, true, PS>(d, Yp, Xp, Zp, Xa, Za, wave * nsw, nsw, q, acc, par);
    else cpass_wave<KW, true, false, PS>(d, Yp, Xp, Zp, Xa, Za, wave * nsw, nsw, q, acc, par);
#pragma unroll
    for (int g = 0; g < 4; ++g) {
        const int rho = q + 4 * g;
#pragma unroll
        for (int ta = 0; ta < 2; ++ta) {
            if (PS) {
                red[wave][2 * rho + ta][2 * r + par] = acc[ta][0][g];
            } else {
#pragma unroll
                for (int tb = 0; tb < 2; ++tb) red[wave][2 * rho + ta][2 * r + tb] = acc[ta][tb][g];
            }
        }
    }
    __syncthreads();
    static_assert(CP_WAVES == 4, "tsum is the canonical tree over four waves");
    auto tsum = [&](int a, int b) { return (red[0][a][b] + red[1][a][b]) + (red[2][a][b] + red[3][a][b]); };
    if (KW > KP && isE) {
        double *Em = E + (size_t)m * KW * KW;
        for (int e = threadIdx.x; e < 32 * 32; e += 64 * CP_WAVES) {
            const int a = e >> 5, b = e & 31, R = 32 * te + a, Cc = 32 * kt + b;
            if ((R >> 4) <= (Cc >> 4)) Em[etile_index(KW / 16, R, Cc)] = tsum(a, b);
        }
        return;
    }
    double *out = isE ? (E + (size_t)m * KW * KW + (size_t)(32 * te) * KW + 32 * kt)
                      : (C + ((size_t)m * d.PP + c0) * KW + 32 * kt);
    if (PS) {
        for (int e = threadIdx.x; e < 32 * 16; e += 64 * CP_WAVES) {
            const int a = e >> 4, b = 2 * (e & 15) + par;
            out[(size_t)a * KW + b] = tsum(a, b);
        }
        return;
    }
    for (int e = threadIdx.x; e < 32 * 32; e += 64 * CP_WAVES) {
        const int a = e >> 5, b = e & 31;
        out[(size_t)a * KW + b] = tsum(a, b);
    }
}


template <int KW>
__global__ __launch_bounds__(256) void k_colsum(Dims d, const double *__restrict__ cpart, double *__restrict__ sloc) {
    __shared__ double smem[8 * 32];
    colsum_tile<KW>(d, cpart, sloc, blockIdx.x, blockIdx.y, smem);
}

__global__ __launch_bounds__(64) void k_delta(Dims d, const double *__restrict__ sall,
                                               const double *__restrict__ delta_in,
                                               const double *__restrict__ tau_in,
                                               double *__restrict__ delta_out,
                                               double *__restrict__ tau_out,
                                               DrawsDev dr,
                                               int64_t iter) {
    delta_shard<KP>(d, sall, delta_in, tau_in, delta_out, tau_out, dr, iter, blockIdx.x, threadIdx.x);
}

__device__ __forceinline__ double tree8(const double (&v)[8]) {
    return ((v[0] + v[1]) + (v[2] + v[3])) + ((v[4] + v[5]) + (v[6] + v[7]));
}

__device__ __forceinline__ void wcol_body(const Dims &d, const Bufs &b, const DrawsDev &dr, int64_t iter, int ops, int colsum,
                                          int wpass, unsigned long long ops_epoch, int xchol, const LamGen &lg,
                                          double *smem) {
    const int G = d.G, nxs = xsum_blocks(G), chunk = G / nxs;
    unsigned long long *chunk_ctr = b.sync + 2;
    int blk = blockIdx.x;
    if (ops) {
        if (blk < G) {
            prep_gram<true>(d, b.Lam, b.omega, b.A, b.ZM, blk, smem);
            WSTAMP(2);
            signal_count(chunk_ctr + blk / chunk);
            prep_ops<true>(d, b.ZM, blk, smem);
            signal_count(b.sync + SYNC_ZM + blk);
            return;
        }
        blk -= G;
    }
    if (colsum) {
        if (blk < G) {
            colsum_tile<KP>(d, b.cpart, b.sloc, blk, 0, smem);
            return;
        }
        blk -= G;
    }
    if (ops) {
        if (blk < nxs) {
            const int t = threadIdx.x, j = blk, m0 = j * chunk;
            constexpr int NU = KP * KP / 256;
            wait_count(chunk_ctr + j, ops_epoch * (unsigned long long)chunk);
            double vs[NU];
            if (chunk <= 8) {
                double v[NU][8];
#pragma unroll
                for (int u = 0; u < NU; ++u)
#pragma unroll
                    for (int U = 0; U < 8; ++U)
                        v[u][U] = (U < chunk) ? ld_agent(b.A + (size_t)(m0 + U) * KP * KP + t + 256 * u) : 0.0;
#pragma unroll
                for (int u = 0; u < NU; ++u) vs[u] = tree8(v[u]);
            } else {
#pragma unroll
                for (int u = 0; u < NU; ++u) {
                    TreeSum<double, 6> ts;
                    for (int k = 0; k < chunk; k += 8) {
                        double v[8];
#pragma unroll
                        for (int U = 0; U < 8; ++U) v[U] = ld_agent(b.A + (size_t)(m0 + k + U) * KP * KP + t + 256 * u);
                        ts.push(tree8(v));
                    }
                    vs[u] = ts.total();
                }
            }
            if (nxs > 1) {
#pragma unroll
                for (int u = 0; u < NU; ++u) st_agent(b.xpart + (size_t)j * KP * KP + t + 256 * u, vs[u]);
                if (!last_arrival(b.ticket, (unsigned)nxs, reinterpret_cast<unsigned *>(smem))) return;
            }
            double xs[NU];
            if (nxs <= 8) {
                double v[NU][8];
#pragma unroll
                for (int u = 0; u < NU; ++u)
#pragma unroll
                    for (int U = 0; U < 8; ++U)
                        v[u][U] = (U < nxs) ? (U == j ? vs[u] : ld_agent(b.xpart + (size_t)U * KP * KP + t + 256 * u))
                                            : 0.0;
#pragma unroll
                for (int u = 0; u < NU; ++u) xs[u] = tree8(v[u]);
            } else {
#pragma unroll
                for (int u = 0; u < NU; ++u) {
                    TreeSum<double, 8> ts;
                    for (int k = 0; k < nxs; k += 8) {
                        double v[8];
#pragma unroll
                        for (int U = 0; U < 8; ++U)
                            v[U] = (k + U < nxs) ? (k + U == j ? vs[u] : ld_agent(b.xpart + (size_t)(k + U) * KP * KP + t + 256 * u))
                                                 : 0.0;
                        static_for<8>([&](auto U) { if (k + U < nxs) ts.push(v[U]); });
                    }
                    xs[u] = ts.total();
                }
            }
            if (!xchol) {
#pragma unroll
                for (int u = 0; u < NU; ++u) b.xa[t + 256 * u] = xs[u];
                return;
            }
            __syncthreads();
#pragma unroll
            for (int u = 0; u < NU; ++u) xprec_store(d, smem, t + 256 * u, xs[u]);
            __syncthreads();
            xchol_factor(d, b.XM, smem);
            return;
        }
        blk -= nxs;
    }
    if (wpass) {
        const int nw = (d.NP / (64 * (3 - wpass))) * d.G;
        if (blk < nw) {
            if (wpass == 2) wpass_z_tile<1>(d, b, dr, iter, xcd_remap(blk, nw), ops_epoch, smem);
            else wpass_z_tile<2>(d, b, dr, iter, xcd_remap(blk, nw), ops_epoch, smem);
            return;
        }
        blk -= nw;
    }
    if (blk < lg.b_total) lam_draws(d, lg, iter, blk * LAM_GEN_THREADS + (int)threadIdx.x, lg.b_total * LAM_GEN_THREADS);
}

#ifndef DCFM_WCOL_WPE
#define DCFM_WCOL_WPE 3
#endif
__global__ __launch_bounds__(256) __attribute__((amdgpu_waves_per_eu(DCFM_WCOL_WPE))) void k_wcol(Dims d, Bufs b, DrawsDev dr, int64_t iter, int ops, int colsum,
                                              int wpass, unsigned long long ops_epoch, int xchol, LamGen lg) {
    __shared__ double smem[PREP_SMEM];
#ifdef DCFM_WSTAMPS
    const unsigned long long t0 = __builtin_amdgcn_s_memrealtime(), c0 = __builtin_readcyclecounter();
#endif
    wcol_body(d, b, dr, iter, ops, colsum, wpass, ops_epoch, xchol, lg, smem);
#ifdef DCFM_WSTAMPS
    if (wpass && threadIdx.x == 0 && blockIdx.x < 8192) {
        g_wstamps[blockIdx.x][0] = t0;
        g_wstamps[blockIdx.x][1] = __builtin_amdgcn_s_memrealtime();
        g_wstamps[blockIdx.x][6] = c0;
        g_wstamps[blockIdx.x][7] = __builtin_readcyclecounter();
    }
#endif
}

__global__ __launch_bounds__(256) void k_eta(Dims d, const double *__restrict__ X,
                                             const double *__restrict__ Z, double *__restrict__ eta) {
    const size_t total = (size_t)d.G * d.NP * d.kp;
    for (size_t e = blockIdx.x * (size_t)blockDim.x + threadIdx.x; e < total;
         e += (size_t)gridDim.x * blockDim.x) {
        const size_t ik = e % ((size_t)d.NP * d.kp);
        eta[e] = eta_of(d.sr, d.s1r, X[ik], Z[e]);
    }
}

template <bool GAMMAS>
__global__ __launch_bounds__(256) void k_draws(Dims d, DrawsDev dr, int64_t iter) {
    const DrawPlan pl = draw_plan(d);
    draws_block<GAMMAS>(d, dr, iter, pl, blockIdx.x + (GAMMAS ? 0 : pl.b_gpsi));
}

__global__ __launch_bounds__(256) void k_rng_fill(uint64_t seed, int kind, double shape, int site,
                                                  int shard, int64_t iter, int64_t count, int width,
                                                  double *__restrict__ out) {
    const Rng rng(seed);
    for (int64_t e = blockIdx.x * (int64_t)blockDim.x + threadIdx.x; e < count;
         e += (int64_t)gridDim.x * blockDim.x) {
        const uint32_t row = (uint32_t)(e / width), k = (uint32_t)(e % width);
        out[e] = kind == 0 ? rng.normal(site, shard, row, k, (uint32_t)iter)
                           : rng.gamma(shape, site, shard, row, k, (uint32_t)iter);
    }
}

void launch_prep(const Dims &d, const Bufs &b, hipStream_t s) {
    if (d.kp != KP) return wide::launch_prep(d, b, s);
    hipLaunchKernelGGL(k_prep, dim3(d.G), dim3(256), 0, s, d, b.Lam, b.omega, b.A, b.ZM);
}
void launch_wpass(const Dims &d, const Bufs &b, hipStream_t s) {
    const dim3 grid((d.NP / 128) * d.G * (d.kp / 32));
    switch (d.kp) {
    case 32: hipLaunchKernelGGL(k_wpass<32>, grid, dim3(256), 0, s, d, b.Y, b.Lam, b.omega, b.W); break;
    case 64: hipLaunchKernelGGL(k_wpass<64>, grid, dim3(256), 0, s, d, b.Y, b.Lam, b.omega, b.W); break;
    default: hipLaunchKernelGGL(k_wpass<128>, grid, dim3(256), 0, s, d, b.Y, b.Lam, b.omega, b.W); break;
    }
}
void launch_zdraw(const Dims &d, const Bufs &b, const DrawsDev &dr, int64_t iter, hipStream_t s) {
    if (d.kp != KP) return wide::launch_zdraw(d, b, dr, iter, s);
    if ((d.NP / ZROWS) * d.G < 256)
        hipLaunchKernelGGL(k_zdraw<256>, dim3((d.NP / 64) * d.G), dim3(256), 0, s, d, b.W, b.ZM, b.X, b.Z, b.Sp, dr, iter);
    else
        hipLaunchKernelGGL(k_zdraw<ZTHREADS>, dim3((d.NP / ZROWS) * d.G), dim3(ZTHREADS), 0, s, d, b.W, b.ZM, b.X, b.Z,
                           b.Sp, dr, iter);
}
void launch_wcol(const Dims &d, const Bufs &b, const DrawsDev &dr, int64_t iter, bool ops, bool colsum, bool wpass,
                 unsigned long long ops_epoch, hipStream_t s, bool lamgen) {
    static_assert(LAM_GEN_THREADS == 256, "k_wcol blocks are 256 threads");
    LamGen lg = {};
    if (lamgen && b.ldraw) lg = lam_gen_plan(d, b.ldraw);
    const int wmode = (d.NP / 128) * d.G <= 256 ? 2 : 1;
    const int nb = (ops ? d.G + xsum_blocks(d.G) : 0) + (colsum ? d.G : 0) + (wpass ? (d.NP / (64 * (3 - wmode))) * d.G : 0);
    if (nb + lg.b_total == 0) return;
    hipLaunchKernelGGL(k_wcol, dim3(nb + lg.b_total), dim3(256), 0, s, d, b, dr, iter, ops ? 1 : 0, colsum ? 1 : 0,
                       wpass ? wmode : 0, ops_epoch, d.coll ? 0 : 1, lg);
}
void launch_xred(const Dims &d, const Bufs &b, hipStream_t s) {
    const int total = d.NP * d.kp;
    hipLaunchKernelGGL(k_xred, dim3(cdiv(total, 256)), dim3(256), 0, s, d, b.Sp, b.xin);
}
void launch_asum(const Dims &d, const Bufs &b, hipStream_t s) {
    hipLaunchKernelGGL(k_asum, dim3(cdiv(d.kp * d.kp, 256)), dim3(256), 0, s, d, b.A, b.xa);
}
void launch_xchol(const Dims &d, const Bufs &b, hipStream_t s) {
    if (d.kp != KP) return wide::launch_xchol(d, b, s);
    hipLaunchKernelGGL(k_xchol, dim3(1), dim3(256), 0, s, d, d.coll ? b.xa_all : b.xa, b.XM);
}
void launch_xdraw(const Dims &d, const Bufs &b, const DrawsDev &dr, int64_t iter, hipStream_t s,
                  bool from_shards) {
    if (d.kp != KP) return wide::launch_xdraw(d, b, dr, iter, s);
    const dim3 grid(cdiv(d.n, XD_ROWS));
    const size_t st = (size_t)d.NP * KP;
    if (from_shards)
        hipLaunchKernelGGL(k_xdraw, grid, dim3(1024), 0, s, d, b.Sp, d.G, st, b.XM, b.X, dr, iter, 0, nullptr, nullptr,
                           0ull);
    else
        hipLaunchKernelGGL(k_xdraw, grid, dim3(1024), 0, s, d, b.xall, d.nranks, st, b.XM, b.X, dr, iter, 0, nullptr,
                           nullptr, 0ull);
}
void launch_xdraw_mr(const Dims &d, const Bufs &b, const DrawsDev &dr, int64_t iter, unsigned long long xm_epoch,
                     hipStream_t s) {
    hipLaunchKernelGGL(k_xdraw, dim3(1 + cdiv(d.n, XD_ROWS)), dim3(1024), 0, s, d, b.xall, d.nranks, (size_t)d.xstride,
                       b.XM, b.X, dr, iter, 1, b.xa_all, b.sync, xm_epoch);
}
void launch_cpass(const Dims &d, const Bufs &b, hipStream_t s, const DrawsDev &dr, const double *delta_in,
                  const double *tau_in, double *delta_out, double *tau_out, int64_t delta_iter) {
    const dim3 grid(((d.PP + d.kp) / 32) * d.G * (d.kp / 32));
    DeltaArgs da;
    da.delta_in = delta_in; da.tau_in = tau_in; da.delta_out = delta_out; da.tau_out = tau_out;
    da.iter = delta_iter;
    const int ndel = (delta_in && d.kp == KP) ? cdiv(d.g, CP_WAVES) : 0;
    switch (d.kp) {
    case 32:
        if (grid.x < 128)
            hipLaunchKernelGGL((k_cpass<32, true>), dim3(2 * grid.x + ndel), dim3(64 * CP_WAVES), 0, s, d, b.Y,
                               b.X, b.Z, b.C, b.E, dr, b.sall, da, ndel);
        else
            hipLaunchKernelGGL((k_cpass<32, false>), dim3(grid.x + ndel), dim3(64 * CP_WAVES), 0, s, d, b.Y, b.X,
                               b.Z, b.C, b.E, dr, b.sall, da, ndel);
        break;
    case 64:
        launch_eta(d, b, b.W, s);
        hipLaunchKernelGGL(k_cpass<64>, grid, dim3(256), 0, s, d, b.Y, b.W, b.Z, b.C, b.E, dr, b.sall, da, 0);
        break;
    default:
        launch_eta(d, b, b.W, s);
        hipLaunchKernelGGL(k_cpass<128>, grid, dim3(256), 0, s, d, b.Y, b.W, b.Z, b.C, b.E, dr, b.sall, da, 0);
        break;
    }
}
void launch_lambda(const Dims &d, const Bufs &b, const DrawsDev &dr, int64_t iter,
                   const double *tau_cur, const double *plam_src, hipStream_t s, bool gen, double kappa_max,
                   const SaveArgs &sv) {
    if (d.kp != KP) return wide::launch_lambda(d, b, dr, iter, tau_cur, plam_src, s, kappa_max);
    const LamDraws ld = lam_draws_at(d, b, dr, iter, gen);
    const dim3 grid(cdiv(d.P, LAM_ROWS), d.G);
#define LAUNCH_LAM(KE)                                                                                       \
    hipLaunchKernelGGL(k_lambda<KE>, grid, dim3(64), 0, s, d, b.C, b.E, b.yy, tau_cur, b.Lam, b.psi, plam_src, \
                       b.ps, b.omega, b.cpart, ld, b.Y, b.X, b.Z, kappa_max, sv)
    if (d.K <= 8) LAUNCH_LAM(8);
    else if (d.K <= 16) LAUNCH_LAM(16);
    else if (d.K <= 20) LAUNCH_LAM(20);
    else if (d.K <= 24) LAUNCH_LAM(24);
    else if (d.K <= 30) LAUNCH_LAM(30);
    else LAUNCH_LAM(32);
#undef LAUNCH_LAM
}
void launch_colsum(const Dims &d, const Bufs &b, hipStream_t s) {
    const dim3 grid(d.G, d.kp / 32);
    switch (d.kp) {
    case 32: hipLaunchKernelGGL(k_colsum<32>, grid, dim3(256), 0, s, d, b.cpart, b.sloc); break;
    case 64: hipLaunchKernelGGL(k_colsum<64>, grid, dim3(256), 0, s, d, b.cpart, b.sloc); break;
    default: hipLaunchKernelGGL(k_colsum<128>, grid, dim3(256), 0, s, d, b.cpart, b.sloc); break;
    }
}
void launch_delta(const Dims &d, const Bufs &b, const DrawsDev &dr, int64_t iter,
                  const double *delta_in, const double *tau_in, double *delta_out, double *tau_out,
                  hipStream_t s) {
    if (d.kp != KP) return wide::launch_delta(d, b, dr, iter, delta_in, tau_in, delta_out, tau_out, s);
    hipLaunchKernelGGL(k_delta, dim3(d.g), dim3(64), 0, s, d, b.sall, delta_in, tau_in, delta_out,
                       tau_out, dr, iter);
}
void launch_eta(const Dims &d, const Bufs &b, double *eta_out, hipStream_t s) {
    const size_t total = (size_t)d.G * d.NP * d.kp;
    const int grid = (int)std::min<size_t>((total + 255) / 256, 8192);
    hipLaunchKernelGGL(k_eta, dim3(grid), dim3(256), 0, s, d, b.X, b.Z, eta_out);
}
void launch_draws(const Dims &d, const DrawsDev &dr, int64_t iter, hipStream_t s) {
    const DrawPlan pl = draw_plan(d);
    hipLaunchKernelGGL(k_draws<true>, dim3(pl.b_gpsi), dim3(256), 0, s, d, dr, iter);
    hipLaunchKernelGGL(k_draws<false>, dim3(pl.total - pl.b_gpsi), dim3(256), 0, s, d, dr, iter);
}
void launch_rng_fill(uint64_t seed, int kind, double shape, int site, int shard, int64_t iter,
                     int64_t count, int width, double *out, hipStream_t s) {
    const int grid = (int)std::min<int64_t>((count + 255) / 256, 8192);
    hipLaunchKernelGGL(k_rng_fill, dim3(grid > 0 ? grid : 1), dim3(256), 0, s, seed, kind, shape, site,
                       shard, iter, count, width, out);
}

__device__ __forceinline__ bool bad(double v) { return !(fabs(v) <= 1.7976931348623157e308); }
__global__ __launch_bounds__(256) void k_finite(Dims d, const double *__restrict__ Lam,
                                                const double *__restrict__ ps, const double *__restrict__ omega,
                                                const double *__restrict__ X, const double *__restrict__ tau,
                                                int *__restrict__ flag) {
    const size_t nL = (size_t)d.G * d.PP * d.kp, nP = (size_t)d.G * d.PP, nX = (size_t)d.NP * d.kp,
                 nT = (size_t)d.g * d.kp;
    bool any = false;
    for (size_t e = blockIdx.x * (size_t)256 + threadIdx.x; e < nL; e += (size_t)gridDim.x * 256) any |= bad(Lam[e]);
    for (size_t e = blockIdx.x * (size_t)256 + threadIdx.x; e < nP; e += (size_t)gridDim.x * 256)
        any |= bad(ps[e]) || bad(omega[e]);
    for (size_t e = blockIdx.x * (size_t)256 + threadIdx.x; e < nX; e += (size_t)gridDim.x * 256) any |= bad(X[e]);
    for (size_t e = blockIdx.x * (size_t)256 + threadIdx.x; e < nT; e += (size_t)gridDim.x * 256) any |= bad(tau[e]);
    if (any) *flag = 1;
}
void launch_finite(const Dims &d, const Bufs &b, const double *tau_cur, int *flag, hipStream_t s) {
    hipLaunchKernelGGL(k_finite, dim3(128), dim3(256), 0, s, d, b.Lam, b.ps, b.omega, b.X, tau_cur, flag);
}

__global__ __launch_bounds__(256) void k_sum_slices(const double *__restrict__ src, int ns, size_t count,
                                                   double *__restrict__ dst) {
    for (size_t i = blockIdx.x * (size_t)256 + threadIdx.x; i < count; i += (size_t)gridDim.x * 256) {
        double v = 0.0;
        for (int k = 0; k < ns; ++k) v += src[(size_t)k * count + i];
        dst[i] = v;
    }
}
void launch_sum_slices(const double *src, int ns, size_t count, double *dst, hipStream_t s) {
    const int grid = (int)std::min<size_t>((count + 255) / 256, 8192);
    hipLaunchKernelGGL(k_sum_slices, dim3(grid > 0 ? grid : 1), dim3(256), 0, s, src, ns, count, dst);
}

}
```

### a-divide-and-conquer-strategy-for-high-dimensional-bayesian-factor-models_amd/csrc/wstamp.h

```cpp
#pragma once
#include <hip/hip_runtime.h>

namespace dcfm {

#ifdef DCFM_WSTAMPS
__device__ unsigned long long g_wstamps[8192][8];
extern "C" int dcfm_debug_wstamps(unsigned long long *out, int nblocks) {
    return (int)hipMemcpyFromSymbol(out, HIP_SYMBOL(g_wstamps), (size_t)nblocks * 64, 0, hipMemcpyDeviceToHost);
}
#define WSTAMP(s) do { if (threadIdx.x == 0 && blockIdx.x < 8192) g_wstamps[blockIdx.x][s] = __builtin_amdgcn_s_memrealtime(); } while (0)
#else
#define WSTAMP(s) do { } while (0)
#endif

}
```

### a-divide-and-conquer-strategy-for-high-dimensional-bayesian-factor-models_amd/csrc/ypass.h

```cpp
#pragma once
#include "dcfm_internal.h"
#include "linalg.h"

namespace dcfm {

#ifndef DCFM_WP_RING
#define DCFM_WP_RING 3
#endif
constexpr int WP_RING = DCFM_WP_RING;
#ifndef DCFM_WP_RING_WIDE
#define DCFM_WP_RING_WIDE 4
#endif
constexpr int WP_RING_WIDE = DCFM_WP_RING_WIDE;
#ifndef DCFM_WP_SKIP_PAD
#define DCFM_WP_SKIP_PAD 1
#endif
constexpr bool WP_SKIP_PAD = DCFM_WP_SKIP_PAD;
template <int KW, int MT, int R = (KW > KP ? WP_RING_WIDE : WP_RING), class Pre>
__device__ __forceinline__ void wpass_acc(const Dims &d, const double *__restrict__ Y, const double *__restrict__ Lam,
                                          const double *__restrict__ omega, int m, int i0, int kt, d4 (&acc)[MT][2],
                                          Pre &&pre) {
    const int lane = threadIdx.x & 63;
    const int r = lane & 15, q = lane >> 4;
    const double *Y0 = Y + ((size_t)m * d.NP + i0 + r) * d.PP + 2 * q;
    const double *Y1 = Y0 + (size_t)16 * (MT - 1) * d.PP;
    const double *L = Lam + (size_t)m * d.PP * KW + 32 * kt + 2 * r;
    const double *wp = omega + (size_t)m * d.PP + 2 * q;
#pragma unroll
    for (int a = 0; a < MT; ++a)
#pragma unroll
        for (int b = 0; b < 2; ++b) acc[a][b] = d4{0.0, 0.0, 0.0, 0.0};
    const int nch = WP_SKIP_PAD ? (d.P + 7) >> 3 : d.PP >> 3;
    d2 y0[R], y1[R], ww[R], l0[R], l1[R];
    auto load = [&](int t, int k) {
        const int j = 8 * t;
        y0[k] = *reinterpret_cast<const d2 *>(Y0 + j);
        if (MT == 2) y1[k] = *reinterpret_cast<const d2 *>(Y1 + j);
        ww[k] = *reinterpret_cast<const d2 *>(wp + j);
        l0[k] = *reinterpret_cast<const d2 *>(L + (size_t)(j + 2 * q) * KW);
        l1[k] = *reinterpret_cast<const d2 *>(L + (size_t)(j + 2 * q + 1) * KW);
    };
    d4 acc2[MT][2];
#pragma unroll
    for (int a = 0; a < MT; ++a)
#pragma unroll
        for (int b = 0; b < 2; ++b) acc2[a][b] = d4{0.0, 0.0, 0.0, 0.0};
    auto mma = [&](int k) {
        const double b00 = ww[k].x * l0[k].x, b01 = ww[k].x * l0[k].y;
        const double b10 = ww[k].y * l1[k].x, b11 = ww[k].y * l1[k].y;
        acc[0][0] = mfma16x16x4(b00, y0[k].x, acc[0][0]);
        acc[0][1] = mfma16x16x4(b01, y0[k].x, acc[0][1]);
        if (MT == 2) {
            acc[MT - 1][0] = mfma16x16x4(b00, y1[k].x, acc[MT - 1][0]);
            acc[MT - 1][1] = mfma16x16x4(b01, y1[k].x, acc[MT - 1][1]);
        }
        acc2[0][0] = mfma16x16x4(b10, y0[k].y, acc2[0][0]);
        acc2[0][1] = mfma16x16x4(b11, y0[k].y, acc2[0][1]);
        if (MT == 2) {
            acc2[MT - 1][0] = mfma16x16x4(b10, y1[k].y, acc2[MT - 1][0]);
            acc2[MT - 1][1] = mfma16x16x4(b11, y1[k].y, acc2[MT - 1][1]);
        }
    };
#pragma unroll
    for (int k = 0; k < R - 1; ++k)
        if (k < nch) load(k, k);
    pre();
    for (int t = 0; t < nch; t += R) {
#pragma unroll
        for (int k = 0; k < R; ++k) {
            if (t + k + R - 1 < nch) load(t + k + R - 1, (k + R - 1) % R);
            if (t + k < nch) mma(k);
        }
    }
#pragma unroll
    for (int a = 0; a < MT; ++a)
#pragma unroll
        for (int b = 0; b < 2; ++b) acc[a][b] += acc2[a][b];
}

template <int KW, int MT = 2>
__device__ __forceinline__ void wpass_tile(const Dims &d, const double *__restrict__ Y,
                                           const double *__restrict__ Lam, const double *__restrict__ omega,
                                           double *__restrict__ W, int w, int kt) {
    const int nrb = d.NP / (64 * MT);
    const int m = w / nrb, rb = w % nrb;
    const int wave = threadIdx.x >> 6, lane = threadIdx.x & 63;
    const int i0 = rb * 64 * MT + wave * 16 * MT;
    const int r = lane & 15, q = lane >> 4;
    d4 acc[MT][2];
    wpass_acc<KW, MT>(d, Y, Lam, omega, m, i0, kt, acc, [] {});
#pragma unroll
    for (int a = 0; a < MT; ++a) {
        double *Wt = W + ((size_t)m * d.NP + i0 + 16 * a + r) * KW + 32 * kt + 2 * q;
#pragma unroll
        for (int g = 0; g < 4; ++g) {
            d2 v;
            v.x = acc[a][0][g];
            v.y = acc[a][1][g];
            *reinterpret_cast<d2 *>(Wt + 8 * g) = v;
        }
    }
}

template <int KW, bool IS_E, bool SAME_T, bool PS = false>
__device__ __forceinline__ void cpass_wave(const Dims &d, const double *__restrict__ Yp,
                                           const double *__restrict__ Xp,
                                           const double *__restrict__ Zp,
                                           const double *__restrict__ Xa,
                                           const double *__restrict__ Za, int s0, int nsw,
                                           int q, d4 (&acc)[2][2], int par = 0) {
    constexpr bool EXTRA = IS_E && !SAME_T, ETA = KW > KP;
    d2 yA[4], xA[4], zA[4], yB[4], xB[4], zB[4];
    auto load = [&](int s, d2 (&y)[4], d2 (&x)[4], d2 (&z)[4]) {
#pragma unroll
        for (int u = 0; u < 4; ++u) {
            const int i = 4 * (s + u) + q;
            x[u] = *reinterpret_cast<const d2 *>(Xp + (size_t)i * KW);
            if (!ETA) z[u] = *reinterpret_cast<const d2 *>(Zp + (size_t)i * KW);
            if (!IS_E) {
                y[u] = *reinterpret_cast<const d2 *>(Yp + (size_t)i * d.PP);
            } else if (EXTRA) {
                const d2 xa = *reinterpret_cast<const d2 *>(Xa + (size_t)i * KW);
                if (ETA) {
                    y[u] = xa;
                } else {
                    const d2 za = *reinterpret_cast<const d2 *>(Za + (size_t)i * KW);
                    y[u].x = eta_of(d.sr, d.s1r, xa.x, za.x);
                    y[u].y = eta_of(d.sr, d.s1r, xa.y, za.y);
                }
            }
        }
    };
    auto mma = [&](d2 (&y)[4], d2 (&x)[4], d2 (&z)[4]) {
#pragma unroll
        for (int u = 0; u < 4; ++u) {
            const double e0 = ETA ? x[u].x : eta_of(d.sr, d.s1r, x[u].x, z[u].x);
            const double e1 = ETA ? x[u].y : eta_of(d.sr, d.s1r, x[u].y, z[u].y);
            const double a0 = (IS_E && SAME_T) ? e0 : y[u].x, a1 = (IS_E && SAME_T) ? e1 : y[u].y;
            if constexpr (PS) {
                const double ep = par ? e1 : e0;
                acc[0][0] = mfma16x16x4(a0, ep, acc[0][0]);
                acc[1][0] = mfma16x16x4(a1, ep, acc[1][0]);
            } else {
                acc[0][0] = mfma16x16x4(a0, e0, acc[0][0]);
                acc[0][1] = mfma16x16x4(a0, e1, acc[0][1]);
                acc[1][0] = mfma16x16x4(a1, e0, acc[1][0]);
                acc[1][1] = mfma16x16x4(a1, e1, acc[1][1]);
            }
        }
    };
    const int nb = nsw >> 2;
    load(s0, yA, xA, zA);
    for (int b = 0; b < nb; b += 2) {
        if (b + 1 < nb) load(s0 + 4 * (b + 1), yB, xB, zB);
        mma(yA, xA, zA);
        if (b + 2 < nb) load(s0 + 4 * (b + 2), yA, xA, zA);
        if (b + 1 < nb) mma(yB, xB, zB);
    }
}

}
```

### include/dcfm.h

```cpp
#ifndef DCFM_H
#define DCFM_H

#include <stdint.h>

#ifdef __cplusplus
extern "C" {
#endif

#define DCFM_ABI_VERSION 2

#define DCFM_OK              0
#define DCFM_ERR_INVALID     1
#define DCFM_ERR_UNSUPPORTED 2
#define DCFM_ERR_HIP         3
#define DCFM_ERR_RCCL        4
#define DCFM_ERR_NUMERIC     5
#define DCFM_ERR_ALLOC       6

#define DCFM_FLAG_INJECT_DRAWS 0x1u
#define DCFM_FLAG_UNFUSED      0x2u
#define DCFM_FLAG_ONE_STREAM   0x4u
#define DCFM_FLAG_FLAT_PRIORITY 0x8u
#define DCFM_FLAG_COMM_SELF    0x20u
#define DCFM_FLAG_EXACT_RESIDUAL 0x10u
#define DCFM_FLAG_GUARD_ALL    0x40u
#define DCFM_FLAG_SIGMA_M2     0x80u
#define DCFM_FLAG_PRECISION_MEAN 0x100u
#define DCFM_FLAG_PARTIAL_CORR 0x200u

typedef struct dcfm_handle dcfm_handle;

typedef struct {
    int32_t n;
    int32_t P;
    int32_t g;
    int32_t K;
    double  rho;
    int64_t burnin;
    int64_t mcmc;
    int64_t thin;
    double  as_, bs, df, ad1, bd1, ad2, bd2;
    uint64_t seed;
    int32_t nranks;
    int32_t rank;
    int32_t device;
    uint32_t flags;
    int32_t asm_batch;
    int32_t reserved[7];
} dcfm_config;

typedef struct {
    double *Lambda;
    double *ps;
    double *omega;
    double *psi;
    double *Plam;
    double *X;
    double *Z;
    double *eta;
    double *delta;
    double *tauh;
} dcfm_state_view;

typedef struct {
    const double *NZ, *NX, *NL, *Gpsi, *Gdelta, *Gps;
} dcfm_draws_view;

int  dcfm_create(const dcfm_config *cfg, dcfm_handle **out);
void dcfm_destroy(dcfm_handle *h);
const char *dcfm_last_error(const dcfm_handle *h);
int  dcfm_abi_version(void);

int  dcfm_comm_unique_id(uint8_t out[128]);
int  dcfm_comm_init(dcfm_handle *h, const uint8_t id[128]);
int  dcfm_comm_init_loopback(dcfm_handle *const *handles, int32_t n);

int  dcfm_set_data(dcfm_handle *h, const double *Yd_local);
int  dcfm_set_data_raw(dcfm_handle *h, const double *Y, int64_t p_in, const int64_t *cols,
                       double *sd_out, double *dev_ms);
int  dcfm_get_data(dcfm_handle *h, double *Yd_local);
int  dcfm_count_nonzero_columns(int device, const double *Y, int32_t n, int64_t p, int32_t *nnz_out,
                                double *dev_ms);
int  dcfm_set_state(dcfm_handle *h, const dcfm_state_view *s);
int  dcfm_init_state(dcfm_handle *h);
int  dcfm_set_draws(dcfm_handle *h, const dcfm_draws_view *d, int64_t first_iter, int64_t n_iter);

int  dcfm_run(dcfm_handle *h, int64_t first_iter, int64_t n_iter);
int  dcfm_synchronize(dcfm_handle *h);

int  dcfm_get_state(dcfm_handle *h, dcfm_state_view *out);
int  dcfm_get_state_raw(dcfm_handle *h, dcfm_state_view *out);
int  dcfm_get_sigma(dcfm_handle *h, double *out);
int  dcfm_get_sigma_cols(dcfm_handle *h, int64_t col0, int64_t ncols, double *out);
int  dcfm_sigma_block(const dcfm_handle *h, int64_t out[3]);
int64_t dcfm_saved_samples(const dcfm_handle *h);
#define DCFM_SIGMA_MEAN 0
#define DCFM_SIGMA_M2   1
#define DCFM_SIGMA_SD   2
int  dcfm_get_sigma_moment_cols(dcfm_handle *h, int32_t which, int64_t col0, int64_t ncols, double *out);
int  dcfm_get_sigma_moment(dcfm_handle *h, int32_t which, double *out);
int  dcfm_get_precision_mean_cols(dcfm_handle *h, int64_t col0, int64_t ncols, double *out);
int  dcfm_get_precision_mean(dcfm_handle *h, double *out);
int  dcfm_get_partial_corr_cols(dcfm_handle *h, int32_t which, int64_t col0, int64_t ncols, double *out);
int  dcfm_get_partial_corr(dcfm_handle *h, int32_t which, double *out);
int  dcfm_sigma_error(dcfm_handle *h, const double *U, int32_t r, const double *s, int32_t iters,
                      uint64_t seed, double out[3]);

int  dcfm_sigma_apply(dcfm_handle *h, const double *V, int32_t nv, double *out, double *dev_ms);
int  dcfm_sigma_eigs(dcfm_handle *h, int32_t r, double tol, int32_t max_passes, uint64_t seed,
                     double *evals, double *evecs, double *resid, int32_t *passes);
int  dcfm_sigma_solve(dcfm_handle *h, const double *B, int32_t nv, double tol, int32_t max_iter,
                      double *X, double *relres, int32_t *iters, double *quad, double *dev_ms);

int  dcfm_set_trace(dcfm_handle *h, int64_t capacity);
int  dcfm_get_trace(dcfm_handle *h, double *out, int64_t *count);

int  dcfm_set_probes(dcfm_handle *h, const double *V, int32_t nv, int64_t capacity);
int  dcfm_get_probe_draws(dcfm_handle *h, double *out, int64_t *count);

int  dcfm_set_precision_probes(dcfm_handle *h, const double *V, int32_t nv, int64_t capacity);
int  dcfm_get_precision_draws(dcfm_handle *h, double *Q, double *logdet, int64_t *count);

int  dcfm_set_loglik(dcfm_handle *h, int64_t capacity);
int  dcfm_get_loglik(dcfm_handle *h, double *maha, double *logdet, int64_t *count);

int  dcfm_set_predict(dcfm_handle *h, const double *Ynew, const uint8_t *observed, int32_t nt, int64_t capacity);
int  dcfm_get_predict(dcfm_handle *h, double *mean, double *m2, double *cvar, double *maha, double *logdet,
                      int64_t *count);

int  dcfm_set_missing(dcfm_handle *h, const uint8_t *mask_local, int64_t capacity);
int  dcfm_get_imputed(dcfm_handle *h, double *mean, double *m2, double *nvar, int64_t *count);

#define DCFM_K_PREP     0
#define DCFM_K_WPASS    1
#define DCFM_K_ZDRAW    2
#define DCFM_K_XRED     3
#define DCFM_K_XDRAW    4
#define DCFM_K_CPASS    5
#define DCFM_K_LAMBDA   6
#define DCFM_K_COLSUM   7
#define DCFM_K_DELTA    8
#define DCFM_K_SAVE     9
#define DCFM_K_ASSEMBLE 10
#define DCFM_K_COMM     11
#define DCFM_K_XCHOL    12
#define DCFM_K_DRAWS    13
#define DCFM_K_RESID    14
#define DCFM_K_COUNT    15
int  dcfm_set_profiling(dcfm_handle *h, int enable);
int  dcfm_set_profiling_mask(dcfm_handle *h, uint32_t mask);
int  dcfm_set_profiling_stride(dcfm_handle *h, int32_t stride);
int  dcfm_get_kernel_stats(dcfm_handle *h, double ms[DCFM_K_COUNT], int64_t launches[DCFM_K_COUNT]);
const char *dcfm_kernel_name(int id);

int  dcfm_rng_fill(int device, uint64_t seed, int kind, double shape, int32_t site,
                   int32_t shard, int64_t iter, int64_t count, double *out);
int  dcfm_rng_fill_rows(int device, uint64_t seed, int kind, double shape, int32_t site,
                        int32_t shard, int64_t iter, int64_t rows, int32_t width, int64_t count,
                        double *out);

#ifdef __cplusplus
}
#endif
#endif
```

Before: 5692 iter/s.

## Fuse X draw into cpass kernel with spread-counter handoff and prefetch

Result: slower. 5485 iter/s (-3.6%).

```diff
diff --git a/a-divide-and-conquer-strategy-for-high-dimensional-bayesian-factor-models_amd/_abi.py b/a-divide-and-conquer-strategy-for-high-dimensional-bayesian-factor-models_amd/_abi.py
--- a/a-divide-and-conquer-strategy-for-high-dimensional-bayesian-factor-models_amd/_abi.py
+++ b/a-divide-and-conquer-strategy-for-high-dimensional-bayesian-factor-models_amd/_abi.py
@@ -24,6 +24,7 @@
 DCFM_FLAG_SIGMA_M2 = 0x80
 DCFM_FLAG_PRECISION_MEAN = 0x100
 DCFM_FLAG_PARTIAL_CORR = 0x200
+DCFM_FLAG_SPLIT_XDRAW = 0x400
 DCFM_SIGMA_MEAN = 0
 DCFM_SIGMA_M2 = 1
 DCFM_SIGMA_SD = 2
diff --git a/a-divide-and-conquer-strategy-for-high-dimensional-bayesian-factor-models_amd/csrc/dcfm.hip b/a-divide-and-conquer-strategy-for-high-dimensional-bayesian-factor-models_amd/csrc/dcfm.hip
--- a/a-divide-and-conquer-strategy-for-high-dimensional-bayesian-factor-models_amd/csrc/dcfm.hip
+++ b/a-divide-and-conquer-strategy-for-high-dimensional-bayesian-factor-models_amd/csrc/dcfm.hip
@@ -499,6 +499,11 @@
     hipStream_t s;
     bool delta_pending = false;
     const DrawsDev &draws() const { return d.inject ? h->dr : h->gen[0]; }
+    bool merged_xdraw() const {
+        const uint32_t timed = (1u << DCFM_K_XDRAW) | (1u << DCFM_K_CPASS);
+        return !d.coll && cpass_draws_x(d) && !(h->cfg.flags & DCFM_FLAG_SPLIT_XDRAW) &&
+               !(h->prof && (h->prof_mask & timed));
+    }
 
     int step(int64_t it) {
         const DrawsDev &dr = draws();
@@ -509,7 +514,8 @@
             KTimer t(h, DCFM_K_COMM, s);
             TRY(coll_allgather(h, CH_MAIN, b.sloc, b.msg_all, (size_t)d.xstride, s));
         }
-        {
+        const bool xride = merged_xdraw();
+        if (!xride) {
             KTimer t(h, DCFM_K_XDRAW, s);
             if (d.coll) launch_xdraw_mr(d, b, dr, it, ++h->xm_ops, s);
             else launch_xdraw(d, b, dr, it, s, true);
@@ -517,8 +523,9 @@
         {
             KTimer t(h, DCFM_K_CPASS, s);
             const DeltaTau dt = delta_tau(h);
-            if (delta_pending) launch_cpass(d, b, s, dr, dt.delta_in, dt.tau_in, dt.delta_out, dt.tau_out, it - 1);
-            else launch_cpass(d, b, s);
+            const unsigned long long xe = xride ? ++h->xr_ops : 0ull;
+            if (delta_pending) launch_cpass(d, b, s, dr, dt.delta_in, dt.tau_in, dt.delta_out, dt.tau_out, it - 1, it, xe);
+            else launch_cpass(d, b, s, dr, nullptr, nullptr, nullptr, nullptr, 0, it, xe);
         }
         HIPC(h, hipGetLastError());
         if (delta_pending) iteration_done(h);
diff --git a/a-divide-and-conquer-strategy-for-high-dimensional-bayesian-factor-models_amd/csrc/dcfm_internal.h b/a-divide-and-conquer-strategy-for-high-dimensional-bayesian-factor-models_amd/csrc/dcfm_internal.h
--- a/a-divide-and-conquer-strategy-for-high-dimensional-bayesian-factor-models_amd/csrc/dcfm_internal.h
+++ b/a-divide-and-conquer-strategy-for-high-dimensional-bayesian-factor-models_amd/csrc/dcfm_internal.h
@@ -134,7 +134,9 @@
 struct PartialCorr {
     double *PC, *PC2;
 };
-constexpr int SYNC_ZM = 2 + 256;
+constexpr int XRIDE_COPIES = 8, XRIDE_PITCH = 32;
+constexpr int SYNC_XRIDE = 2 + 256;
+constexpr int SYNC_ZM = SYNC_XRIDE + XRIDE_COPIES * XRIDE_PITCH;
 __host__ __device__ inline int xsum_blocks(int G) {
     if (G <= XSUM_BLOCKS) return 1;
     int chunk = 1;
@@ -172,9 +174,11 @@
 void launch_xchol(const Dims &d, const Bufs &b, hipStream_t s);
 void launch_xdraw(const Dims &d, const Bufs &b, const DrawsDev &dr, int64_t iter, hipStream_t s,
                   bool from_shards = false);
+bool cpass_draws_x(const Dims &d);
 void launch_cpass(const Dims &d, const Bufs &b, hipStream_t s, const DrawsDev &dr = DrawsDev{},
                   const double *delta_in = nullptr, const double *tau_in = nullptr, double *delta_out = nullptr,
-                  double *tau_out = nullptr, int64_t delta_iter = 0);
+                  double *tau_out = nullptr, int64_t delta_iter = 0, int64_t x_iter = 0,
+                  unsigned long long x_epoch = 0);
 void launch_lambda(const Dims &d, const Bufs &b, const DrawsDev &dr, int64_t iter,
                    const double *tau_cur, const double *plam_src, hipStream_t s, bool gen, double kappa_max,
                    const SaveArgs &sv = SaveArgs{});
diff --git a/a-divide-and-conquer-strategy-for-high-dimensional-bayesian-factor-models_amd/csrc/handle.h b/a-divide-and-conquer-strategy-for-high-dimensional-bayesian-factor-models_amd/csrc/handle.h
--- a/a-divide-and-conquer-strategy-for-high-dimensional-bayesian-factor-models_amd/csrc/handle.h
+++ b/a-divide-and-conquer-strategy-for-high-dimensional-bayesian-factor-models_amd/csrc/handle.h
@@ -44,6 +44,7 @@
     bool plam_valid = false;
     unsigned long long wc_ops = 0;
     unsigned long long xm_ops = 0;
+    unsigned long long xr_ops = 0;
     bool asm_pending[2] = {false, false};
     int cur = 0;
     int lb = 0;
diff --git a/a-divide-and-conquer-strategy-for-high-dimensional-bayesian-factor-models_amd/csrc/handoff.h b/a-divide-and-conquer-strategy-for-high-dimensional-bayesian-factor-models_amd/csrc/handoff.h
--- a/a-divide-and-conquer-strategy-for-high-dimensional-bayesian-factor-models_amd/csrc/handoff.h
+++ b/a-divide-and-conquer-strategy-for-high-dimensional-bayesian-factor-models_amd/csrc/handoff.h
@@ -25,6 +25,17 @@
     __syncthreads();
 }
 
+__device__ __forceinline__ void signal_count_spread(unsigned long long *ctr, int copies, int pitch) {
+    stores_done();
+    if ((int)threadIdx.x < copies)
+        __hip_atomic_fetch_add(ctr + threadIdx.x * pitch, 1ull, __ATOMIC_RELAXED, __HIP_MEMORY_SCOPE_AGENT);
+}
+__device__ __forceinline__ void wait_count_slow(unsigned long long *ctr, unsigned long long target) {
+    if (threadIdx.x == 0)
+        while (__hip_atomic_load(ctr, __ATOMIC_RELAXED, __HIP_MEMORY_SCOPE_AGENT) < target) __builtin_amdgcn_s_sleep(16);
+    __syncthreads();
+}
+
 __device__ __forceinline__ bool last_arrival(unsigned *ticket, unsigned count, unsigned *flag) {
     stores_done();
     if (threadIdx.x == 0) {
diff --git a/a-divide-and-conquer-strategy-for-high-dimensional-bayesian-factor-models_amd/csrc/kernels.hip b/a-divide-and-conquer-strategy-for-high-dimensional-bayesian-factor-models_amd/csrc/kernels.hip
--- a/a-divide-and-conquer-strategy-for-high-dimensional-bayesian-factor-models_amd/csrc/kernels.hip
+++ b/a-divide-and-conquer-strategy-for-high-dimensional-bayesian-factor-models_amd/csrc/kernels.hip
@@ -79,6 +79,171 @@
 constexpr bool XD_SPREAD = DCFM_XD_SPREAD;
 constexpr int XD_LDS = 2 * KP * (KP + 1) + 4 * 4 * 64 * 2 + 4 * 64 * 2;
 constexpr int XD_SMEM = XD_LDS > XCHOL_SMEM ? XD_LDS : XCHOL_SMEM;
+template <int CW, bool PUB>
+__device__ __forceinline__ void xdraw_rows(const Dims &d, const double *__restrict__ src, int nsrc, size_t stride,
+                                           const double *XM, double *X, const DrawsDev &dr, int64_t iter, int blk,
+                                           double *smem, int xroles, unsigned long long *xm_ctr,
+                                           unsigned long long xm_target) {
+    constexpr int NT = 256 * CW, NJ = 4 / CW, NXM = 2 * KP * KP / NT;
+    static_assert(CW == 1 || CW == 4, "four column groups x CW chunk waves");
+    double (*Ms)[KP][KP + 1] = reinterpret_cast<double (*)[KP][KP + 1]>(smem);
+    d2 (*part)[4][64] = reinterpret_cast<d2 (*)[4][64]>(smem + 2 * KP * (KP + 1));
+    d2 (*evs)[64] = reinterpret_cast<d2 (*)[64]>(smem + 2 * KP * (KP + 1) + CW * 4 * 64 * 2);
+    const int lane = threadIdx.x & 63, w = threadIdx.x >> 6, c = lane & 15, q = lane >> 4;
+    const int tw = w & 3, sw = w >> 2;
+    const int i0 = blk * XD_ROWS, i = i0 + c;
+    const bool live = c < XD_ROWS && i < d.n;
+    int nch, chunk;
+    xdraw_chunks(nsrc, nch, chunk);
+    d2 sv[4], ev[4];
+    if (w == 0 && d.inject) {
+        const double *nx = dr.NX + ((size_t)(iter - dr.first_iter) * d.n + (live ? i : 0)) * d.K;
+#pragma unroll
+        for (int t = 0; t < 4; ++t) {
+            const int kk = 8 * t + 2 * q;
+            ev[t].x = (live && kk < d.K) ? nx[kk] : 0.0;
+            ev[t].y = (live && kk + 1 < d.K) ? nx[kk + 1] : 0.0;
+        }
+    } else if (w == 0 && !XD_SPREAD) {
+        const Rng rng(d.seed);
+#pragma unroll
+        for (int t = 0; t < 4; ++t) {
+            const int kk = 8 * t + 2 * q;
+            double n0 = 0.0, n1 = 0.0;
+            if (live && kk < d.K) rng.normal2(SITE_X, 0u, (uint32_t)i, (uint32_t)(4 * t + q), (uint32_t)iter, n0, n1);
+            ev[t].x = n0;
+            ev[t].y = (kk + 1 < d.K) ? n1 : 0.0;
+        }
+    }
+    double xmv[NXM];
+#pragma unroll
+    for (int u = 0; u < NXM; ++u) xmv[u] = 0.0;
+    if (!(xroles & 1)) {
+#pragma unroll
+        for (int u = 0; u < NXM; ++u) xmv[u] = XM[threadIdx.x + NT * u];
+    }
+    auto draw = [&] {
+        if (!XD_SPREAD || d.inject || w >= 4) return;
+        const int kk = 8 * w + 2 * q;
+        double n0 = 0.0, n1 = 0.0;
+        if (live && kk < d.K) Rng(d.seed).normal2(SITE_X, 0u, (uint32_t)i, (uint32_t)(4 * w + q), (uint32_t)iter, n0, n1);
+        evs[w][lane] = d2{n0, (kk + 1 < d.K) ? n1 : 0.0};
+    };
+    d2 pv[NJ];
+    if (chunk >= 2) {
+        constexpr int NPART = 16 / XD_ROWS;
+        const int np = (chunk & (chunk - 1)) ? 1 : (chunk < NPART ? chunk : NPART), per = chunk / np;
+        const int rr = c % XD_ROWS, h = c / XD_ROWS;
+        const bool rl = i0 + rr < d.n && h < np;
+        const double *p0 = src + (size_t)((h < np ? h : 0) * per) * stride +
+                           (size_t)(i0 + rr < d.n ? i0 + rr : i0) * KP + 8 * tw + 2 * q;
+        if (NJ > 1 && per <= 4) {
+            d2 v[NJ][4];
+            static_for<NJ>([&](auto J) {
+                const double *p = p0 + (size_t)(J * chunk) * stride;
+                static_for<4>([&](auto U) {
+                    if (J < nch && U < per) v[J][U] = rl ? *reinterpret_cast<const d2 *>(p + (size_t)U * stride) : d2{0.0, 0.0};
+                });
+            });
+            draw();
+            static_for<NJ>([&](auto J) {
+                TreeSum<d2, 3> ts;
+                static_for<4>([&](auto U) { if (J < nch && U < per) ts.push(v[J][U]); });
+                pv[J] = J < nch ? ts.total() : d2{0.0, 0.0};
+            });
+        } else {
+            static_for<NJ>([&](auto J) {
+                const int s = sw + CW * J;
+                pv[J] = d2{0.0, 0.0};
+                if (s < nch) {
+                    const double *p = p0 + (size_t)(s * chunk) * stride;
+                    pv[J] = tree_sum_f<d2, 8, 10>(per, [&](int rk) {
+                        return rl ? *reinterpret_cast<const d2 *>(p + (size_t)rk * stride) : d2{0.0, 0.0};
+                    }, [&] { if (J == 0) draw(); });
+                }
+            });
+        }
+        static_for<NJ>([&](auto J) {
+            d2 v = pv[J];
+            for (int o = 1; o < np; o <<= 1) {
+                d2 u;
+                u.x = __shfl_down(v.x, o * XD_ROWS, 16);
+                u.y = __shfl_down(v.y, o * XD_ROWS, 16);
+                v.x = v.x + u.x;
+                v.y = v.y + u.y;
+            }
+            pv[J] = h == 0 ? v : d2{0.0, 0.0};
+        });
+    } else {
+        const double *p0 = src + (size_t)(live ? i : i0) * KP + 8 * tw + 2 * q;
+        static_for<NJ>([&](auto J) {
+            const int s = sw + CW * J;
+            pv[J] = (s < nch && live) ? *reinterpret_cast<const d2 *>(p0 + (size_t)(s * chunk) * stride) : d2{0.0, 0.0};
+        });
+        draw();
+    }
+    if (PUB) CSTAMP(6);
+    if (CW == 1) {
+        TreeSum<d2, 3> ts;
+        static_for<NJ>([&](auto J) { if (J < nch) ts.push(pv[J]); });
+        part[0][tw][lane] = ts.total();
+    } else if (sw < nch) {
+        part[sw][tw][lane] = pv[0];
+    }
+    if (xroles & 1) {
+        wait_count(xm_ctr, xm_target);
+#pragma unroll
+        for (int u = 0; u < NXM; ++u) xmv[u] = ld_agent(XM + threadIdx.x + NT * u);
+    }
+#pragma unroll
+    for (int u = 0; u < NXM; ++u) {
+        const int e = threadIdx.x + NT * u;
+        const int mat = e / (KP * KP), rem = e % (KP * KP);
+        Ms[mat][rem / KP][rem % KP] = xmv[u];
+    }
+    __syncthreads();
+    if (w > 0) return;
+    if (XD_SPREAD && !d.inject) {
+#pragma unroll
+        for (int t = 0; t < 4; ++t) ev[t] = evs[t][lane];
+    }
+#pragma unroll
+    for (int t = 0; t < 4; ++t) {
+        if (CW == 1) {
+            sv[t] = part[0][t][lane];
+        } else {
+            TreeSum<d2, 3> ts;
+            for (int k = 0; k < nch; ++k) ts.push(part[k][t][lane]);
+            sv[t] = ts.total();
+        }
+    }
+    d4 ax[2];
+    ax[0] = ax[1] = d4{0.0, 0.0, 0.0, 0.0};
+#pragma unroll
+    for (int t = 0; t < 4; ++t)
+#pragma unroll
+        for (int e = 0; e < 2; ++e) {
+            const int kk = 8 * t + 2 * q + e;
+            const double se = e ? sv[t].y : sv[t].x, ee = e ? ev[t].y : ev[t].x;
+#pragma unroll
+            for (int mt = 0; mt < 2; ++mt) {
+                ax[mt] = mfma16x16x4(Ms[0][16 * mt + c][kk], se, ax[mt]);
+                ax[mt] = mfma16x16x4(Ms[1][16 * mt + c][kk], ee, ax[mt]);
+            }
+        }
+    if (PUB) CSTAMP(7);
+    if (!live) return;
+    double *Xr = X + (size_t)i * KP;
+#pragma unroll
+    for (int mt = 0; mt < 2; ++mt)
+#pragma unroll
+        for (int g = 0; g < 4; ++g) {
+            const int k = 16 * mt + q + 4 * g;
+            const double v = (k < d.K) ? ax[mt][g] : 0.0;
+            if (PUB) st_agent(Xr + k, v);
+            else Xr[k] = v;
+        }
+}
 __global__ __launch_bounds__(1024) void k_xdraw(Dims d, const double *__restrict__ src, int nsrc, size_t sstride,
                                                 double *__restrict__ XM,
                                                 double *__restrict__ X, DrawsDev dr, int64_t iter, int xroles,
@@ -97,140 +262,52 @@
         }
         blk -= 1;
     }
-    double (*Ms)[KP][KP + 1] = reinterpret_cast<double (*)[KP][KP + 1]>(smem);
-    d2 (*part)[4][64] = reinterpret_cast<d2 (*)[4][64]>(smem + 2 * KP * (KP + 1));
-    d2 (*evs)[64] = reinterpret_cast<d2 (*)[64]>(smem + 2 * KP * (KP + 1) + 4 * 4 * 64 * 2);
-    const int lane = threadIdx.x & 63, w = threadIdx.x >> 6, c = lane & 15, q = lane >> 4;
-    const int tw = w & 3, sw = w >> 2;
-    const int i0 = blk * XD_ROWS, i = i0 + c;
-    const bool live = c < XD_ROWS && i < d.n;
-    const size_t stride = sstride;
-    int nch, chunk;
-    xdraw_chunks(nsrc, nch, chunk);
-    d2 sv[4], ev[4];
-    if (w == 0 && d.inject) {
-        const double *nx = dr.NX + ((size_t)(iter - dr.first_iter) * d.n + (live ? i : 0)) * d.K;
-#pragma unroll
-        for (int t = 0; t < 4; ++t) {
-            const int kk = 8 * t + 2 * q;
-            ev[t].x = (live && kk < d.K) ? nx[kk] : 0.0;
-            ev[t].y = (live && kk + 1 < d.K) ? nx[kk + 1] : 0.0;
-        }
-    } else if (w == 0 && !XD_SPREAD) {
-        const Rng rng(d.seed);
-#pragma unroll
-        for (int t = 0; t < 4; ++t) {
-            const int kk = 8 * t + 2 * q;
-            double n0 = 0.0, n1 = 0.0;
-            if (live && kk < d.K) rng.normal2(SITE_X, 0u, (uint32_t)i, (uint32_t)(4 * t + q), (uint32_t)iter, n0, n1);
-            ev[t].x = n0;
-            ev[t].y = (kk + 1 < d.K) ? n1 : 0.0;
-        }
-    }
-    double xmv[2] = {0.0, 0.0};
-    if (!(xroles & 1)) {
-#pragma unroll
-        for (int u = 0; u < 2; ++u) xmv[u] = XM[threadIdx.x + 1024 * u];
-    }
-    auto draw = [&] {
-        if (!XD_SPREAD || d.inject || w >= 4) return;
-        const int kk = 8 * w + 2 * q;
-        double n0 = 0.0, n1 = 0.0;
-        if (live && kk < d.K) Rng(d.seed).normal2(SITE_X, 0u, (uint32_t)i, (uint32_t)(4 * w + q), (uint32_t)iter, n0, n1);
-        evs[w][lane] = d2{n0, (kk + 1 < d.K) ? n1 : 0.0};
-    };
-    if (sw < nch) {
-        if (chunk >= 2) {
-            constexpr int NPART = 16 / XD_ROWS;
-            const int np = (chunk & (chunk - 1)) ? 1 : (chunk < NPART ? chunk : NPART), per = chunk / np;
-            const int rr = c % XD_ROWS, h = c / XD_ROWS;
-            const bool rl = i0 + rr < d.n && h < np;
-            const double *p = src + (size_t)(sw * chunk + (h < np ? h : 0) * per) * stride +
-                              (size_t)(i0 + rr < d.n ? i0 + rr : i0) * KP + 8 * tw + 2 * q;
-            d2 v = tree_sum_f<d2, 8, 10>(per, [&](int rk) {
-                return rl ? *reinterpret_cast<const d2 *>(p + (size_t)rk * stride) : d2{0.0, 0.0};
-            }, draw);
-            for (int o = 1; o < np; o <<= 1) {
-                d2 u;
-                u.x = __shfl_down(v.x, o * XD_ROWS, 16);
-                u.y = __shfl_down(v.y, o * XD_ROWS, 16);
-                v.x = v.x + u.x;
-                v.y = v.y + u.y;
-            }
-            part[sw][tw][lane] = h == 0 ? v : d2{0.0, 0.0};
-        } else {
-            const double *p = src + (size_t)sw * chunk * stride + (size_t)(live ? i : i0) * KP + 8 * tw + 2 * q;
-            const d2 v = live ? *reinterpret_cast<const d2 *>(p) : d2{0.0, 0.0};
-            draw();
-            part[sw][tw][lane] = v;
-        }
-    }
-    if (xroles & 1) {
-        wait_count(xm_ctr, xm_target);
-#pragma unroll
-        for (int u = 0; u < 2; ++u) xmv[u] = ld_agent(XM + threadIdx.x + 1024 * u);
-    }
-#pragma unroll
-    for (int u = 0; u < 2; ++u) {
-        const int e = threadIdx.x + 1024 * u;
-        const int mat = e / (KP * KP), rem = e % (KP * KP);
-        Ms[mat][rem / KP][rem % KP] = xmv[u];
-    }
-    __syncthreads();
-    if (w > 0) return;
-    if (XD_SPREAD && !d.inject) {
-#pragma unroll
-        for (int t = 0; t < 4; ++t) ev[t] = evs[t][lane];
-    }
-#pragma unroll
-    for (int t = 0; t < 4; ++t) {
-        TreeSum<d2, 3> ts;
-        for (int k = 0; k < nch; ++k) ts.push(part[k][t][lane]);
-        sv[t] = ts.total();
-    }
-    d4 ax[2];
-    ax[0] = ax[1] = d4{0.0, 0.0, 0.0, 0.0};
-#pragma unroll
-    for (int t = 0; t < 4; ++t)
-#pragma unroll
-        for (int e = 0; e < 2; ++e) {
-            const int kk = 8 * t + 2 * q + e;
-            const double se = e ? sv[t].y : sv[t].x, ee = e ? ev[t].y : ev[t].x;
-#pragma unroll
-            for (int mt = 0; mt < 2; ++mt) {
-                ax[mt] = mfma16x16x4(Ms[0][16 * mt + c][kk], se, ax[mt]);
-                ax[mt] = mfma16x16x4(Ms[1][16 * mt + c][kk], ee, ax[mt]);
-            }
-        }
-    if (!live) return;
-    double *Xr = X + (size_t)i * KP;
-#pragma unroll
-    for (int mt = 0; mt < 2; ++mt)
-#pragma unroll
-        for (int g = 0; g < 4; ++g) {
-            const int k = 16 * mt + q + 4 * g;
-            Xr[k] = (k < d.K) ? ax[mt][g] : 0.0;
-        }
+    xdraw_rows<4, false>(d, src, nsrc, sstride, XM, X, dr, iter, blk, smem, xroles, xm_ctr, xm_target);
 }
 
 constexpr int CP_WAVES = 4;
+struct XRide {
+    const double *Sp;
+    const double *XM;
+    double *X;
+    unsigned long long *ctr, target;
+    int64_t iter;
+    int nx;
+};
 template <int KW, bool PS = false>
 __global__ __launch_bounds__(64 * CP_WAVES) __attribute__((amdgpu_waves_per_eu(3))) void k_cpass(Dims d, const double *__restrict__ Y,
                                                               const double *__restrict__ X,
                                                               const double *__restrict__ Z,
                                                               double *__restrict__ C, double *__restrict__ E,
                                                               DrawsDev dr, const double *__restrict__ sall,
-                                                              DeltaArgs da, int ndel) {
+                                                              DeltaArgs da, int ndel, XRide xr) {
     __shared__ double red[CP_WAVES][32][33];
+    static_assert(sizeof(red) / sizeof(double) >= 2 * KP * (KP + 1) + 4 * 64 * 2 + 4 * 64 * 2, "xdraw_rows<1>'s LDS");
+    const int nx = KW == KP ? xr.nx : 0;
     const int nbc = gridDim.x - ndel;
+    CSTAMP(0);
     if constexpr (KW == KP) {
         if ((int)blockIdx.x >= nbc) {
             const int m = (blockIdx.x - nbc) * CP_WAVES + (threadIdx.x >> 6);
             if (m < d.g)
                 delta_shard<KP>(d, sall, da.delta_in, da.tau_in, da.delta_out, da.tau_out, dr, da.iter, m, threadIdx.x & 63);
+            CSTAMP(1);
             return;
         }
-    }
+        if ((int)blockIdx.x < nx) {
+            xdraw_rows<1, true>(d, xr.Sp, d.G, (size_t)d.NP * KP, xr.XM, xr.X, dr, xr.iter, blockIdx.x, &red[0][0][0],
+                                0, nullptr, 0ull);
+            signal_count_spread(xr.ctr, XRIDE_COPIES, XRIDE_PITCH);
+            CSTAMP(5);
+        }
+    }
+    auto xwait = [&] {
+        if constexpr (KW == KP) {
+            CSTAMP(2);
+            if (nx) wait_count_slow(xr.ctr + (blockIdx.x & (XRIDE_COPIES - 1)) * XRIDE_PITCH, xr.target);
+            CSTAMP(3);
+        }
+    };
     const int nt = (d.PP + KW) >> 5, nkt = KW / 32;
     int w = xcd_remap(blockIdx.x, nbc);
     const int par = PS ? (w & 1) : 0;
@@ -254,9 +331,10 @@
     for (int a = 0; a < 2; ++a)
 #pragma unroll
         for (int b = 0; b < 2; ++b) acc[a][b] = d4{0.0, 0.0, 0.0, 0.0};
-    if (!isE) cpass_wave<KW, false, false, PS>(d, Yp, Xp, Zp, Xa, Za, wave * nsw, nsw, q, acc, par);
-    else if (te == kt) cpass_wave<KW, true, true, PS>(d, Yp, Xp, Zp, Xa, Za, wave * nsw, nsw, q, acc, par);
-    else cpass_wave<KW, true, false, PS>(d, Yp, Xp, Zp, Xa, Za, wave * nsw, nsw, q, acc, par);
+    if (!isE) cpass_wave<KW, false, false, PS>(d, Yp, Xp, Zp, Xa, Za, wave * nsw, nsw, q, acc, par, xwait);
+    else if (te == kt) cpass_wave<KW, true, true, PS>(d, Yp, Xp, Zp, Xa, Za, wave * nsw, nsw, q, acc, par, xwait);
+    else cpass_wave<KW, true, false, PS>(d, Yp, Xp, Zp, Xa, Za, wave * nsw, nsw, q, acc, par, xwait);
+    CSTAMP(4);
 #pragma unroll
     for (int g = 0; g < 4; ++g) {
         const int rho = q + 4 * g;
@@ -288,12 +366,14 @@
             const int a = e >> 4, b = 2 * (e & 15) + par;
             out[(size_t)a * KW + b] = tsum(a, b);
         }
+        CSTAMP(1);
         return;
     }
     for (int e = threadIdx.x; e < 32 * 32; e += 64 * CP_WAVES) {
         const int a = e >> 5, b = e & 31;
         out[(size_t)a * KW + b] = tsum(a, b);
     }
+    CSTAMP(1);
 }
 
 
@@ -533,29 +613,42 @@
     hipLaunchKernelGGL(k_xdraw, dim3(1 + cdiv(d.n, XD_ROWS)), dim3(1024), 0, s, d, b.xall, d.nranks, (size_t)d.xstride,
                        b.XM, b.X, dr, iter, 1, b.xa_all, b.sync, xm_epoch);
 }
+static int cpass32_tiles(const Dims &d) {
+    const int t = ((d.PP + KP) / 32) * d.G;
+    return t < 128 ? 2 * t : t;
+}
+bool cpass_draws_x(const Dims &d) { return d.kp == KP && cdiv(d.n, XD_ROWS) <= cpass32_tiles(d); }
 void launch_cpass(const Dims &d, const Bufs &b, hipStream_t s, const DrawsDev &dr, const double *delta_in,
-                  const double *tau_in, double *delta_out, double *tau_out, int64_t delta_iter) {
+                  const double *tau_in, double *delta_out, double *tau_out, int64_t delta_iter, int64_t x_iter,
+                  unsigned long long x_epoch) {
     const dim3 grid(((d.PP + d.kp) / 32) * d.G * (d.kp / 32));
     DeltaArgs da;
     da.delta_in = delta_in; da.tau_in = tau_in; da.delta_out = delta_out; da.tau_out = tau_out;
     da.iter = delta_iter;
     const int ndel = (delta_in && d.kp == KP) ? cdiv(d.g, CP_WAVES) : 0;
+    XRide xr = {};
+    if (x_epoch && cpass_draws_x(d)) {
+        xr.Sp = b.Sp; xr.XM = b.XM; xr.X = b.X; xr.ctr = b.sync + SYNC_XRIDE;
+        xr.nx = cdiv(d.n, XD_ROWS);
+        xr.target = x_epoch * (unsigned long long)xr.nx;
+        xr.iter = x_iter;
+    }
     switch (d.kp) {
     case 32:
         if (grid.x < 128)
             hipLaunchKernelGGL((k_cpass<32, true>), dim3(2 * grid.x + ndel), dim3(64 * CP_WAVES), 0, s, d, b.Y,
-                               b.X, b.Z, b.C, b.E, dr, b.sall, da, ndel);
+                               b.X, b.Z, b.C, b.E, dr, b.sall, da, ndel, xr);
         else
             hipLaunchKernelGGL((k_cpass<32, false>), dim3(grid.x + ndel), dim3(64 * CP_WAVES), 0, s, d, b.Y, b.X,
-                               b.Z, b.C, b.E, dr, b.sall, da, ndel);
+                               b.Z, b.C, b.E, dr, b.sall, da, ndel, xr);
         break;
     case 64:
         launch_eta(d, b, b.W, s);
-        hipLaunchKernelGGL(k_cpass<64>, grid, dim3(256), 0, s, d, b.Y, b.W, b.Z, b.C, b.E, dr, b.sall, da, 0);
+        hipLaunchKernelGGL(k_cpass<64>, grid, dim3(256), 0, s, d, b.Y, b.W, b.Z, b.C, b.E, dr, b.sall, da, 0, xr);
         break;
     default:
         launch_eta(d, b, b.W, s);
-        hipLaunchKernelGGL(k_cpass<128>, grid, dim3(256), 0, s, d, b.Y, b.W, b.Z, b.C, b.E, dr, b.sall, da, 0);
+        hipLaunchKernelGGL(k_cpass<128>, grid, dim3(256), 0, s, d, b.Y, b.W, b.Z, b.C, b.E, dr, b.sall, da, 0, xr);
         break;
     }
 }
diff --git a/a-divide-and-conquer-strategy-for-high-dimensional-bayesian-factor-models_amd/csrc/wstamp.h b/a-divide-and-conquer-strategy-for-high-dimensional-bayesian-factor-models_amd/csrc/wstamp.h
--- a/a-divide-and-conquer-strategy-for-high-dimensional-bayesian-factor-models_amd/csrc/wstamp.h
+++ b/a-divide-and-conquer-strategy-for-high-dimensional-bayesian-factor-models_amd/csrc/wstamp.h
@@ -9,8 +9,14 @@
     return (int)hipMemcpyFromSymbol(out, HIP_SYMBOL(g_wstamps), (size_t)nblocks * 64, 0, hipMemcpyDeviceToHost);
 }
 #define WSTAMP(s) do { if (threadIdx.x == 0 && blockIdx.x < 8192) g_wstamps[blockIdx.x][s] = __builtin_amdgcn_s_memrealtime(); } while (0)
+__device__ unsigned long long g_cstamps[2048][8];
+extern "C" int dcfm_debug_cstamps(unsigned long long *out, int nblocks) {
+    return (int)hipMemcpyFromSymbol(out, HIP_SYMBOL(g_cstamps), (size_t)nblocks * 64, 0, hipMemcpyDeviceToHost);
+}
+#define CSTAMP(s) do { if (threadIdx.x == 0 && blockIdx.x < 2048) g_cstamps[blockIdx.x][s] = __builtin_amdgcn_s_memrealtime(); } while (0)
 #else
 #define WSTAMP(s) do { } while (0)
+#define CSTAMP(s) do { } while (0)
 #endif
 
 }
diff --git a/a-divide-and-conquer-strategy-for-high-dimensional-bayesian-factor-models_amd/csrc/ypass.h b/a-divide-and-conquer-strategy-for-high-dimensional-bayesian-factor-models_amd/csrc/ypass.h
--- a/a-divide-and-conquer-strategy-for-high-dimensional-bayesian-factor-models_amd/csrc/ypass.h
+++ b/a-divide-and-conquer-strategy-for-high-dimensional-bayesian-factor-models_amd/csrc/ypass.h
@@ -16,6 +16,10 @@
 #define DCFM_WP_SKIP_PAD 1
 #endif
 constexpr bool WP_SKIP_PAD = DCFM_WP_SKIP_PAD;
+#ifndef DCFM_XRIDE_PREFETCH
+#define DCFM_XRIDE_PREFETCH 1
+#endif
+constexpr bool XRIDE_PREFETCH = DCFM_XRIDE_PREFETCH;
 template <int KW, int MT, int R = (KW > KP ? WP_RING_WIDE : WP_RING), class Pre>
 __device__ __forceinline__ void wpass_acc(const Dims &d, const double *__restrict__ Y, const double *__restrict__ Lam,
                                           const double *__restrict__ omega, int m, int i0, int kt, d4 (&acc)[MT][2],
@@ -102,16 +106,39 @@
     }
 }
 
-template <int KW, bool IS_E, bool SAME_T, bool PS = false>
+template <int KW, bool IS_E, bool SAME_T, bool PS = false, class XWait>
 __device__ __forceinline__ void cpass_wave(const Dims &d, const double *__restrict__ Yp,
                                            const double *__restrict__ Xp,
                                            const double *__restrict__ Zp,
                                            const double *__restrict__ Xa,
                                            const double *__restrict__ Za, int s0, int nsw,
-                                           int q, d4 (&acc)[2][2], int par = 0) {
+                                           int q, d4 (&acc)[2][2], int par, XWait &&xwait) {
     constexpr bool EXTRA = IS_E && !SAME_T, ETA = KW > KP;
     d2 yA[4], xA[4], zA[4], yB[4], xB[4], zB[4];
-    auto load = [&](int s, d2 (&y)[4], d2 (&x)[4], d2 (&z)[4]) {
+    auto load = [&](int s, d2 (&y)[4], d2 (&x)[4], d2 (&z)[4], int part = 3) {
+        if (part != 3) {
+#pragma unroll
+            for (int u = 0; u < 4; ++u) {
+                const int i = 4 * (s + u) + q;
+                if (part == 1) {
+                    if (!ETA) z[u] = *reinterpret_cast<const d2 *>(Zp + (size_t)i * KW);
+                    if (!IS_E) y[u] = *reinterpret_cast<const d2 *>(Yp + (size_t)i * d.PP);
+                } else {
+                    x[u] = *reinterpret_cast<const d2 *>(Xp + (size_t)i * KW);
+                    if (EXTRA) {
+                        const d2 xa = *reinterpret_cast<const d2 *>(Xa + (size_t)i * KW);
+                        if (ETA) {
+                            y[u] = xa;
+                        } else {
+                            const d2 za = *reinterpret_cast<const d2 *>(Za + (size_t)i * KW);
+                            y[u].x = eta_of(d.sr, d.s1r, xa.x, za.x);
+                            y[u].y = eta_of(d.sr, d.s1r, xa.y, za.y);
+                        }
+                    }
+                }
+            }
+            return;
+        }
 #pragma unroll
         for (int u = 0; u < 4; ++u) {
             const int i = 4 * (s + u) + q;
@@ -150,7 +177,14 @@
         }
     };
     const int nb = nsw >> 2;
-    load(s0, yA, xA, zA);
+    if (XRIDE_PREFETCH) {
+        load(s0, yA, xA, zA, 1);
+        xwait();
+        load(s0, yA, xA, zA, 2);
+    } else {
+        xwait();
+        load(s0, yA, xA, zA);
+    }
     for (int b = 0; b < nb; b += 2) {
         if (b + 1 < nb) load(s0 + 4 * (b + 1), yB, xB, zB);
         mma(yA, xA, zA);
diff --git a/include/dcfm.h b/include/dcfm.h
--- a/include/dcfm.h
+++ b/include/dcfm.h
@@ -27,6 +27,7 @@
 #define DCFM_FLAG_SIGMA_M2     0x80u
 #define DCFM_FLAG_PRECISION_MEAN 0x100u
 #define DCFM_FLAG_PARTIAL_CORR 0x200u
+#define DCFM_FLAG_SPLIT_XDRAW  0x400u
 
 typedef struct dcfm_handle dcfm_handle;
 
```
